# TensorSpeech/TensorFlowASR

Measured on AMD Instinct MI355X. Metric: audio-hours/sec (train step) Conformer-M RNN-T, higher is better.
Workload: dtype bf16; 1 GPU; Conformer-M transducer full train step (fwd+RNN-T loss+bwd+Adam), LibriSpeech-shaped 16 kHz utterances, 32/GPU, padding=batch, SpecAugment on, dropout 0.1; global_batch=32, parallelism=dp1, params=32461288

## Files before the change

include/tfasr_hip.h:

```cpp
#ifndef TFASR_HIP_H_
#define TFASR_HIP_H_

#include <stddef.h>
#include <stdint.h>

#ifdef __cplusplus
extern "C" {
#endif

#define TFASR_ABI_VERSION 44

typedef enum {
  TFASR_STATUS_SUCCESS = 0,
  TFASR_STATUS_INVALID_VALUE = 1,
  TFASR_STATUS_EXECUTION_FAILED = 2,
  TFASR_STATUS_UNSUPPORTED = 3
} tfasr_status_t;

typedef enum { TFASR_F32 = 0, TFASR_BF16 = 1 } tfasr_dtype_t;

const char* tfasr_status_string(int status);
int tfasr_abi_version(void);
size_t tfasr_launch_count(void);

// ... 8 lines not shown
int tfasr_rnnt_row_labels(const int32_t* labels, const int32_t* label_len, const int32_t* logit_len, const long* cell_off,
                          long total_cells, int B, int T, int U1, int V, int32_t* row_label, void* stream);
int tfasr_rnnt_loss_packed_stats(const void* logits, void* grads, const int32_t* labels, const int32_t* label_len,
                                 const int32_t* logit_len, const float* grad_scale, const long* cell_off, long total_cells,
                                 const float* lse_part, int lse_parts, const float* pick, int B, int T, int U1, int V, int blank,
                                 int dtype, float* costs, void* workspace, size_t workspace_bytes, void* stream);
int tfasr_rnnt_loss_packed(const void* logits, void* grads, const int32_t* labels, const int32_t* label_len,
                           const int32_t* logit_len, const float* grad_scale, const long* cell_off, long total_cells, int B,
                           int T, int U1, int V, int blank, int dtype, float* costs, void* workspace,
                           size_t workspace_bytes, void* stream);

int tfasr_ctc_loss_workspace_size(int B, int T, int U, int V, size_t* bytes);
int tfasr_ctc_loss(const void* logits, void* grads, const int32_t* labels, const int32_t* label_len,
                   const int32_t* logit_len, const float* grad_scale, int B, int T, int U, int V, int blank, int dtype,
                   float* costs, void* workspace, size_t workspace_bytes, void* stream);
int tfasr_ctc_greedy_decode(const void* logits, const int32_t* logit_len, int32_t* workspace_argmax, int32_t* tokens,
                            int32_t* tokens_len, int B, int T, int V, int blank, int dtype, void* stream);
int tfasr_ctc_greedy_decode_detail(const void* logits, const int32_t* logit_len, int32_t* workspace, int32_t* tokens, int32_t* tokens_len,
                                   int32_t* starts, int32_t* ends, float* tok_logp, float* tok_entropy, float* score, int B, int T, int V,
                                   int blank, int dtype, void* stream);

typedef enum { TFASR_ACT_NONE = 0, TFASR_ACT_SWISH = 1, TFASR_ACT_TANH = 2, TFASR_ACT_SIGMOID = 3, TFASR_ACT_TANH_OUT = 4,
               TFASR_ACT_FACTOR = 5  } tfasr_act_t;

typedef struct {
  const void* A; const void* B; void* D;
  const float* bias;
  const void* res;
  const void* dact_z;
  void* prez;
  int M, N, K;
  int lda, ldb, ldd;
  int trans_a, trans_b;
  int nb1, nb2;
  long sA1, sA2, sB1, sB2, sD1, sD2;
  float alpha, beta;
  int act;
  int dact;
  int dtype;
  int out_f32;
  int accumulate;
  int split_k;
  float drop_p;
  long drop_seed;
  float* ws;
  long ws_elems;
  float* colsum;
  float* lse_part; int lse_parts; const int32_t* row_label; float* pick;
  const long* seg_a_off; const long* seg_b_off; int seg_k;
  const float* rgrad_coef;
  const void* bns_x; const float* bns_fin; float* bns_out; int bns_copies;
  int bns_c;
  const int32_t* row_tiles; int n_row_tiles;
} tfasr_gemm_args;

int tfasr_gemm(const tfasr_gemm_args* args, void* stream);
int tfasr_gemm_group(const tfasr_gemm_args* args, int n, void* stream);

int tfasr_layernorm_fwd(const void* x, const float* gamma, const float* beta, void* y, float* mean, float* rstd,
                        long rows, int C, float eps, int dtype, void* stream);
int tfasr_ffn_fused_fwd(const void* x, const float* gamma, const float* beta, const void* W1, const float* b1, const void* W2,
                        const float* b2, void* y, void* ln, float* mean, float* rstd, void* z, void* h, long rows, int d, int F,
                        float ln_eps, float res_factor, float drop_p, long drop_seed1, long drop_seed2, int dtype, void* stream);
int tfasr_ffn_fused_fwd2(const void* x, const float* gamma, const float* beta, const void* W1, const float* b1, const void* W2,
                         const float* b2, void* y, void* ln, float* mean, float* rstd, void* z, int z_factor, void* h, long rows, int d, int F,
                         float ln_eps, float res_factor, float drop_p, long drop_seed1, long drop_seed2, int dtype, void* stream);
int tfasr_ln_dense_fwd(const void* x, const float* gamma, const float* beta, const void* W, const float* b, void* out, void* ln, float* mean,
                       float* rstd, long rows, int d, int N, float ln_eps, int dtype, void* stream);
int tfasr_layernorm_bwd(const void* dy, const void* x, const float* gamma, const float* mean, const float* rstd,
                        const void* add, void* dx, float* dgamma, float* dbeta, long rows, int C, int dtype,
                        void* stream);
int tfasr_layernorm_bwd_drop(const void* dy, const void* x, const float* gamma, const float* mean, const float* rstd,
                             const void* add, void* dx, float* dgamma, float* dbeta, void* dx_dropped, float drop_p,
                             long drop_seed, long rows, int C, int dtype, void* stream);
int tfasr_layernorm_bwd_part_blocks(long rows, int C, int dtype);
int tfasr_layernorm_bwd_part(const void* dy, const void* x, const float* gamma, const float* mean, const float* rstd, const void* add,
                             void* dx, float* part, void* dx_dropped, float drop_p, long drop_seed, long rows, int C, int dtype,
                             void* stream);
int tfasr_layernorm_bwd_part_n(const void* dy, const void* x, const float* gamma, const float* mean, const float* rstd, const void* add,
                               void* dx, float* part, int nblk, void* dx_dropped, float drop_p, long drop_seed, long rows, int C, int dtype,
                               void* stream);
int tfasr_dense_ln_bwd(const void* dy, const void* W, int K, const void* x, const float* gamma, const float* mean, const float* rstd,
                       const void* add, void* dx, float* part, int nblk, void* dx_dropped, float drop_p, long drop_seed, long rows,
                       int d, float alpha, int dtype, void* stream);
int tfasr_layernorm_bwd_fold(const float* part, int nsets, int nblk, int C, float* const* dgamma, float* const* dbeta, void* stream);
int tfasr_layernorm_bwd_fold_sets(const float* const* part, int nsets, int nblk, int C, float* const* dgamma, float* const* dbeta,
                                  void* stream);
int tfasr_bn_stats(const void* x, float* stats, long rows, int C, int dtype, void* stream);
int tfasr_bn_finalize(const float* stats, float count, const float* gamma, const float* beta, float* fin,
                      float* moving_mean, float* moving_var, float momentum, float eps, int C, int training,
                      void* stream);
int tfasr_bn_finalize_apply_fwd(const void* x, const float* stats, float count, const float* gamma, const float* beta, float* fin,
                                float* moving_mean, float* moving_var, float momentum, float eps, void* y, long rows, int C, int act,
                                int training, int dtype, void* stream);
int tfasr_bn_finalize_apply_fwd_copies(const void* x, const float* stats, int copies, float count, const float* gamma, const float* beta, float* fin,
                                       float* moving_mean, float* moving_var, float momentum, float eps, void* y, long rows, int C, int act,
                                       int training, int dtype, void* stream);
int tfasr_bn_apply_fwd(const void* x, const float* fin, void* y, long rows, int C, int act, int dtype, void* stream);
int tfasr_bn_bwd_stats(const void* x, const void* dy, const float* fin, float* bstats, long rows, int C, int act,
                       int dtype, void* stream);
int tfasr_bn_apply_bwd_grads(const void* x, const void* dy, const float* fin, const float* bstats, float count, void* dx, long rows,
                            int C, int act, float* dgamma, float* dbeta, float grad_scale, int dtype, void* stream);
int tfasr_bn_apply_bwd_grads_copies(const void* x, const void* dy, const float* fin, const float* bstats, int copies, float count, void* dx,
                                    long rows, int C, int act, float* dgamma, float* dbeta, float grad_scale, int dtype, void* stream);
int tfasr_bn_apply_bwd(const void* x, const void* dy, const float* fin, const float* bstats, float count, void* dx,
                       long rows, int C, int act, int dtype, void* stream);
// ... 111 lines not shown
                         void* stream);
int tfasr_decode_step(const float* emb, const float* lstm_k, const float* lstm_rk, const float* lstm_b, const float* ln_g,
                      const float* ln_b, const float* joint_pred_w, const float* joint_pred_b, const float* vocab_w,
                      const float* vocab_b, const float* packed, const float* encj, const int32_t* nframes, const int32_t* frame_idx,
                      const int32_t* tok_idx, const int32_t* prev_tok, const float* h, const float* c, int32_t* active,
                      float* h_new, float* c_new, float* z, float* logits, int B, int T, int E, int P, int J, int V,
                      int max_tokens, int mode, float ln_eps, void* stream);
int tfasr_decode_steps(const float* emb, const float* lstm_k, const float* lstm_rk, const float* lstm_b, const float* ln_g,
                       const float* ln_b, const float* joint_pred_w, const float* joint_pred_b, const float* vocab_w,
                       const float* vocab_b, const float* packed, const float* encj, const int32_t* nframes, int32_t* frame_idx,
                       int32_t* tok_idx, int32_t* prev_tok, float* h, float* c, int32_t* active, float* h_new, float* c_new, float* z,
                       float* logits, int32_t* tokens, int32_t* per_frame, int B, int T, int E, int P, int J, int V, int max_tokens,
                       int blank, int mode, int max_tokens_per_frame, float ln_eps, int iters, void* stream);
size_t tfasr_decode_pack_floats(int E, int P, int J, int V);
int tfasr_decode_pack(const float* emb, const float* lstm_k, const float* lstm_rk, const float* joint_pred_w, const float* vocab_w,
                      float* packed, int E, int P, int J, int V, void* stream);
int tfasr_decode_update(const void* logits, const int32_t* active, const int32_t* nframes, int32_t* frame_idx,
                        int32_t* prev_tok, int32_t* tok_idx, int32_t* tokens, int32_t* per_frame, const void* h_new,
                        const float* c_new, void* h, float* c, int B, int V, int P, int max_tokens, int blank, int mode,
                        int max_tokens_per_frame, int dtype, void* stream);
int tfasr_decode_update_detail(const void* logits, const int32_t* active, const int32_t* nframes, int32_t* frame_idx,
                               int32_t* prev_tok, int32_t* tok_idx, int32_t* tokens, int32_t* per_frame, const void* h_new,
                               const float* c_new, void* h, float* c, int32_t* tok_frames, float* tok_logp, float* tok_entropy, int B,
                               int V, int P, int max_tokens, int blank, int mode, int max_tokens_per_frame, int dtype, void* stream);
int tfasr_decode_steps_detail(const float* emb, const float* lstm_k, const float* lstm_rk, const float* lstm_b, const float* ln_g,
                              const float* ln_b, const float* joint_pred_w, const float* joint_pred_b, const float* vocab_w,
                              const float* vocab_b, const float* packed, const float* encj, const int32_t* nframes, int32_t* frame_idx,
                              int32_t* tok_idx, int32_t* prev_tok, float* h, float* c, int32_t* active, float* h_new, float* c_new,
                              float* z, float* logits, int32_t* tokens, int32_t* per_frame, int32_t* tok_frames, float* tok_logp,
                              float* tok_entropy, int B, int T, int E, int P, int J, int V, int max_tokens, int blank, int mode,
                              int max_tokens_per_frame, float ln_eps, int iters, void* stream);

int tfasr_conv1_fwd(const void* x, const float* w, const float* bias, void* y, int B, int T0, int F0, int C, int dtype,
                    void* stream);
int tfasr_conv1_bwd_weight(const void* x, const void* dy, float* dw, float* db, int B, int T0, int F0, int C,
                           int dtype, void* stream);
int tfasr_conv1_fwd_s2d(const void* x, const float* w, const float* bias, void* y, int B, int T0, int F0, int C, int dtype,
                        void* stream);
int tfasr_conv1_bwd_weight_s2d(const void* x, const void* dy, float* dw, float* db, int B, int T0, int F0, int C, int dtype,
                               void* stream);
int tfasr_conv1_stats(const void* x, const float* w, const float* bias, float* stats, int B, int T0, int F0, int C, int dtype,
                      void* stream);
int tfasr_conv1_bn_apply_s2d(const void* x, const float* w, const float* bias, const float* fin, void* y, int B, int T0, int F0, int C,
                             int dtype, void* stream);
int tfasr_conv1_bn_bwd_stats_s2d(const void* x, const float* w, const float* bias, const float* fin, const void* dy, float* bstats, int B,
                                 int T0, int F0, int C, int dtype, void* stream);
int tfasr_conv1_bn_bwd_apply_s2d(const void* x, const float* w, const float* bias, const float* fin, const float* bstats, float count,
                                 const void* dy, float* dw, float* db, int B, int T0, int F0, int C, int dtype, void* stream);
#define TFASR_CONV1_GRAM_DOUBLES 768
int tfasr_conv1_gram(const void* x, double* gram, int B, int T0, int F0, int dtype, void* stream);
int tfasr_conv1_stats_from_gram(const double* gram, const float* w, const float* bias, float* stats, int C, void* stream);
int tfasr_conv1_bn_bwd_onepass_s2d(const void* x, const float* w, const float* bias, const float* fin, const void* dy, float* bstats,
                                   float* pbuf, int B, int T0, int F0, int C, int dtype, void* stream);
int tfasr_conv1_bn_bwd_finalize(const double* gram, const float* w, const float* bias, const float* fin, const float* bstats, float count,
                                const float* pbuf, float* dw, float* db, int C, void* stream);
int tfasr_halo_zero(void* x, int B, int T2, int F2, int W, int dtype, void* stream);
int tfasr_s2d_edge_zero(void* x, int B, int T1, int F1, int C, int dtype, void* stream);
int tfasr_s2d_tail_fill(void* x, const int32_t* tiles, int n_tiles, const int32_t* rep_tt, int B, int T2, int F2, int C, int dtype,
                        void* stream);
int tfasr_im2col_3x3s2(const void* x, void* col, int B, int T1, int F1, int C, int dtype, void* stream);
int tfasr_col2im_3x3s2(const void* dcol, void* dx, int B, int T1, int F1, int C, int dtype, void* stream);

int tfasr_logmel(const float* signal, int B, int N, float preemph, const float* window, int frame_len, int frame_step,
                 int nfft, const float* melw, const int32_t* band, int F, float eps, void* out, int T0, int dtype,
                 void* stream);

int tfasr_rows_subsample_fwd(const void* x, void* y, int B, int T, int C, int stride, int dtype, void* stream);
int tfasr_rows_subsample_bwd(const void* dy, void* dx, int B, int T, int C, int stride, int dtype, void* stream);
int tfasr_se_pool(const void* x, const int32_t* lengths, float* pool, int B, int T, int C, int dtype, void* stream);
int tfasr_se_scale_fwd(const void* x, const float* scale, void* y, int B, int T, int C, int dtype, void* stream);
int tfasr_se_scale_bwd_reduce(const void* x, const void* dy, float* dscale, int B, int T, int C, int dtype, void* stream);
int tfasr_se_bwd_apply(const void* dy, const float* scale, const float* dpool, const int32_t* lengths, void* dx, int B, int T,
                       int C, int dtype, void* stream);
int tfasr_add_act_fwd(const void* a, const void* b, void* y, long n, int act, int dtype, void* stream);
int tfasr_add_act_bwd(const void* a, const void* b, const void* dy, void* d, long n, int act, int dtype, void* stream);

int tfasr_ctc_beam_search_host(const float* logits, const int32_t* logit_len, int B, int T, int V, int beam_width,
                               int blank_index, int32_t* tokens, int32_t* tokens_len, float* log_prob);

int tfasr_ctc_beam_search_workspace_size(int B, int T, int V, int beam_width, size_t* bytes);
int tfasr_ctc_beam_search(const void* logits, const int32_t* logit_len, int B, int T, int V, int beam_width, int top_paths,
                          int blank_index, int dtype, int32_t* tokens, int32_t* tokens_len, float* log_prob, void* workspace,
                          size_t workspace_bytes, void* stream);

int tfasr_rnnt_beam_workspace_size(int B, int T, int U, int J, int V, int beam_width, size_t* bytes);
int tfasr_rnnt_beam_search(const float* emb, const float* lstm_k, const float* lstm_rk, const float* lstm_b, const float* ln_g,
                           const float* ln_b, const float* joint_pred_w, const float* joint_pred_b, const float* vocab_w,
                           const float* vocab_b, const float* packed, const float* encj, const int32_t* nframes,
                           const int32_t* init_tok, const float* init_h, const float* init_c, int B, int T, int E, int U, int J,
                           int V, int beam_width, int top_paths, int blank, float ln_eps, int32_t* tokens, int32_t* tokens_len,
                           float* score, int32_t* next_tok, float* next_h, float* next_c, void* workspace, size_t workspace_bytes,
                           void* stream);
int tfasr_rnnt_beam_begin(const int32_t* init_tok, int B, int T, int U, int J, int V, int beam_width, int blank, void* workspace,
                          size_t workspace_bytes, void* stream);
int tfasr_rnnt_beam_select(const float* logits, const int32_t* nframes, int t, int B, int T, int U, int J, int V, int beam_width,
                           int blank, void* workspace, size_t workspace_bytes, void* stream);
int tfasr_rnnt_beam_nbest(int B, int T, int U, int J, int V, int beam_width, int top_paths, int blank, int32_t* tokens,
                          int32_t* tokens_len, float* score, void* workspace, size_t workspace_bytes, void* stream);

int tfasr_rnnt_beam_reset(const int32_t* mask, int B, int Tcap, int U, int J, int V, int beam_width, int blank, void* workspace,
                          size_t workspace_bytes, void* stream);
int tfasr_rnnt_beam_advance(const float* emb, const float* lstm_k, const float* lstm_rk, const float* lstm_b, const float* ln_g,
                            const float* ln_b, const float* joint_pred_w, const float* joint_pred_b, const float* vocab_w,
                            const float* vocab_b, const float* packed, const float* encj, const int32_t* nvalid, int B, int C,
                            int Tcap, int E, int U, int J, int V, int beam_width, int blank, float ln_eps, int frames_max_after,
                            void* workspace, size_t workspace_bytes, void* stream);
int tfasr_rnnt_beam_commit(const int32_t* final_mask, int32_t* committed, int32_t* tokens, int32_t* ntokens, int B, int Tcap, int U,
                           int J, int V, int beam_width, int width, int blank, void* workspace, size_t workspace_bytes, void* stream);
int tfasr_rnnt_beam_nbest_states(int B, int Tcap, int U, int J, int V, int beam_width, int top_paths, int blank, int width,
                                 int32_t* tokens, int32_t* tokens_len, float* score, int32_t* next_tok, float* next_h, float* next_c,
                                 void* workspace, size_t workspace_bytes, void* stream);
int tfasr_ctc_beam_stream_workspace_size(int B, int C, int Tcap, int V, int beam_width, size_t* bytes);
// ... 186 lines not shown
```

tensorflowasr_amd/_lib.py:

```python
import ctypes
import os
from ctypes import POINTER, Structure, c_char_p, c_float, c_int, c_int32, c_long, c_size_t, c_void_p

HERE = os.path.dirname(os.path.abspath(__file__))
LIB_PATH = os.environ.get("TFASR_LIB") or os.path.join(HERE, "lib", "libtfasr_hip.so")

TFASR_F32, TFASR_BF16 = 0, 1
ACT_NONE, ACT_SWISH, ACT_TANH, ACT_SIGMOID, ACT_TANH_OUT, ACT_FACTOR = 0, 1, 2, 3, 4, 5


class TfasrError(RuntimeError):
    pass


class GemmArgs(Structure):
    _fields_ = [
        ("A", c_void_p), ("B", c_void_p), ("D", c_void_p),
        ("bias", c_void_p), ("res", c_void_p), ("dact_z", c_void_p), ("prez", c_void_p),
        ("M", c_int), ("N", c_int), ("K", c_int),
        ("lda", c_int), ("ldb", c_int), ("ldd", c_int),
        ("trans_a", c_int), ("trans_b", c_int),
        ("nb1", c_int), ("nb2", c_int),
        ("sA1", c_long), ("sA2", c_long), ("sB1", c_long), ("sB2", c_long), ("sD1", c_long), ("sD2", c_long),
        ("alpha", c_float), ("beta", c_float),
        ("act", c_int), ("dact", c_int), ("dtype", c_int), ("out_f32", c_int), ("accumulate", c_int), ("split_k", c_int),
        ("drop_p", c_float), ("drop_seed", c_long),
        ("ws", c_void_p), ("ws_elems", c_long), ("colsum", c_void_p),
        ("lse_part", c_void_p), ("lse_parts", c_int), ("row_label", c_void_p), ("pick", c_void_p),
        ("seg_a_off", c_void_p), ("seg_b_off", c_void_p), ("seg_k", c_int),
        ("rgrad_coef", c_void_p),
        ("bns_x", c_void_p), ("bns_fin", c_void_p), ("bns_out", c_void_p), ("bns_copies", c_int), ("bns_c", c_int),
        ("row_tiles", c_void_p), ("n_row_tiles", c_int),
    ]


BLOCK_PARAM_NAMES = [
    "ff1/ln/g", "ff1/ln/b", "ff1/d1/w", "ff1/d1/b", "ff1/d2/w", "ff1/d2/b",
    "ff2/ln/g", "ff2/ln/b", "ff2/d1/w", "ff2/d1/b", "ff2/d2/w", "ff2/d2/b",
    "mhsa/ln/g", "mhsa/ln/b", "mhsa/qkv/w", "mhsa/qkv/b", "mhsa/pos/w", "mhsa/pos/b", "mhsa/o/w", "mhsa/o/b", "/enc/u", "/enc/v",
    "conv/ln/g", "conv/ln/b", "conv/pw1/w", "conv/pw1/b", "conv/dw/w", "conv/dw/b", "conv/bn/g", "conv/bn/b", "conv/pw2/w", "conv/pw2/b",
    "ln/g", "ln/b",
]
PHASE_A, PHASE_B = 1, 2


class BlockCfg(Structure):
    _fields_ = [
        ("B", c_int), ("T", c_int), ("d", c_int), ("H", c_int), ("dh", c_int), ("dff", c_int), ("ksize", c_int),
        ("dtype", c_int), ("training", c_int), ("save", c_int), ("use_mask", c_int), ("force_unfused", c_int), ("world", c_int),
        ("site0", c_int), ("drop_epoch", c_long),
        ("drop_p", c_float), ("ffm_res", c_float), ("mhsa_res", c_float), ("conv_res", c_float), ("ln_eps", c_float), ("bn_eps", c_float),
        ("bn_momentum", c_float),
        ("chunk_size", c_int), ("history_size", c_int), ("dw_norm_layer", c_int), ("dh_logical", c_int),
    ]


class BlockParams(Structure):
    _fields_ = [
        ("flat", c_void_p), ("shadow", c_void_p), ("grad", c_void_p), ("bn_mm", c_void_p), ("bn_mv", c_void_p), ("pe", c_void_p),
        ("off", c_long * len(BLOCK_PARAM_NAMES)),
    ]


class BlockIO(Structure):
    _fields_ = [
        ("x_in", c_void_p), ("x_out", c_void_p), ("dy", c_void_p), ("dx", c_void_p), ("lengths", c_void_p),
        ("bn_stats", c_void_p), ("bn_bstats", c_void_p),
        ("stash", c_void_p), ("stash_bytes", c_size_t), ("scratch", c_void_p), ("scratch_bytes", c_size_t),
        ("prezeroed", c_int), ("dpext_zero", c_void_p), ("wgrad_slot", c_int),
        ("pext_pre", c_void_p), ("defer_pos_grad", c_int), ("ln_part_ext", c_void_p), ("ln_part_ext_floats", c_size_t),
        ("dcv_keep", c_void_p), ("ds_keep", c_void_p), ("qv_keep", c_void_p), ("bn_stats_copies", c_int),
    ]


def _parse_header():
    import re

    hdr = os.path.join(HERE, "..", "include", "tfasr_hip.h")
    if not os.path.exists(hdr):
        hdr = os.path.join(HERE, "tfasr_hip.h")
    src = open(hdr).read()
    src = re.sub(r"/\*.*?\*/", "", src, flags=re.S)
    src = re.sub(r"typedef\s+struct\s*\{.*?\}\s*\w+\s*;", "", src, flags=re.S)
    sigs = {}
    for m in re.finditer(r"(const\s+char\s*\*|int|size_t)\s+(tfasr_[a-z0-9_]+)\s*\(([^)]*)\)\s*;", src):
# ... 75 lines not shown
```

tensorflowasr_amd/conformer.py:

```python
import math
import os

import numpy as np
import torch

from . import kernels as K
from .base_model import BaseModel
from .kernels import ACT_NONE, ACT_SWISH, ACT_TANH_OUT
from .params import ParamStore
from .schemas import AlignOutput, PredictInput, PredictOutput, RecognizeOutput, TrainData, TrainInput, TrainOutput


class SingleProcess:

    world = 1
    rank = 0

    def allreduce_stats_(self, t):
        return t

    def set_reduce(self, on):
        pass

    def grads_ready(self, lo, hi):
        pass

    def finish_grads(self):
        pass


def _split_k(M, N, Kd):
    tiles = -(-M // 128) * -(-N // 128)
    if tiles >= 512 or Kd <= 2048:
        return 1
    v = int(max(1, min(-(-1024 // tiles), Kd // 1024, 64)))
    return (v + 4) // 8 * 8 if v >= 12 else v


class ConformerTransducer(BaseModel):
    def __init__(self, cfg, device=None, dtype=torch.bfloat16, seed=0, dp=None):
        if not torch.cuda.is_available():
            raise K._lib.TfasrError("ConformerTransducer needs an MI355X (HIP) device; there is no CPU fallback")
        self.cfg = cfg
        self.device = torch.device("cuda", torch.cuda.current_device()) if device is None else torch.device(device)
        self.dtype = dtype
        pad = (dtype == torch.bfloat16 and cfg.head_size < 64 and getattr(cfg, "encoder", "conformer") == "conformer"
               and os.environ.get("TFASR_HEAD_PAD", "1") != "0")
        cpad = (dtype == torch.bfloat16 and cfg.filters % 64 != 0 and getattr(cfg, "encoder", "conformer") == "conformer"
                and getattr(cfg, "sub_norm", "batch") == "batch" and os.environ.get("TFASR_FILTER_PAD", "1") != "0")
        self.ps = ParamStore(cfg, self.device, dtype, seed, head_phys=64 if pad else None, filt_phys=-(-cfg.filters // 64) * 64 if cpad else None)
        self.dp = dp or SingleProcess()
        self.blank = cfg.blank
        self.time_reduction_factor = cfg.time_reduction_factor
        self.step = 0
        self._consts = {}
        self._bn1_sums_in_gemm = True
        self._bn_stats_copies = 8
        self._conv1_gram = True
        self._sub_tail_once = os.environ.get("TFASR_SUB_TAIL", "1") != "0"
        self._front_tail = None
        self._rng = np.random.default_rng([seed + 1000, int(self.dp.rank)])
        prio = -1
        self.pred_stream = torch.cuda.Stream(device=self.device, priority=prio)
        self.use_pred_stream = os.environ.get("TFASR_NO_PRED_STREAM", "0") != "1"
        self._dp_force_split = os.environ.get("TFASR_DP_FORCE_SPLIT", "0") == "1" and not isinstance(self.dp, SingleProcess)
        self._lstm_persist_auto = os.environ.get("TFASR_LSTM_PERSIST") is None
        self.optimizer = dict(beta1=0.9, beta2=0.98, eps=1e-9, weight_decay=1e-6, schedule=dict(
            dmodel=cfg.dmodel, warmup_steps=10000, scale=2.0, max_lr=0.05 / math.sqrt(cfg.dmodel)))
        self.ga_steps = 1
        self.prefetched_inputs = False
        self._ga_count = 0
        self._drop_epoch = 0
        self.native_blocks = os.environ.get("TFASR_NATIVE_BLOCK", "1") != "0"
        self.wgrad_stream = {"0": False, "1": True}.get(os.environ.get("TFASR_WGRAD_STREAM"), None)
        self._wgrad_keep = []
        self._blk_params, self._blk_sizes = {}, {}
        self._zero_pool = {}
        self.block_hoist = {"0": False, "1": True}.get(os.environ.get("TFASR_BLOCK_HOIST"), None)
        self.dpext_aux = True
        self.joint_wgrad_aux = False
        self._aux_pending = False
        if self.device.type != "cuda":
            self.aux_stream = None
        else:
            with torch.cuda.device(self.device):
                self.aux_stream = torch.cuda.ExternalStream(K.block_side_stream(), device=self.device)
        self._hoisted = {}
        self.fuse_joint_stats = True
        self.joint_recompute = os.environ.get("TFASR_JOINT_RECOMPUTE", "0") == "1"
        self._after_encoder = "pred/emb" if cfg.head == "transducer" else "dec/logits/w"
        self.timers = None
        self.timer_work = {}
        self.time_sections = False
        self.decode_precision = os.environ.get("TFASR_DECODE_PRECISION", "f32")
        self.decode_fused = True
        self._twin = None

    def _frontend_consts(self):
        if "fe" not in self._consts:
            c = self.cfg
            n = c.frame_length
            window = (0.5 - 0.5 * np.cos(2.0 * np.pi * np.arange(n) / n)).astype(np.float32)
            melw = _mel_weight_matrix(c.num_feature_bins, c.nfft // 2 + 1, c.sample_rate, c.lower_edge_hertz, c.upper_edge_hertz)
            band = np.zeros((melw.shape[1], 2), np.int32)
            for m in range(melw.shape[1]):
                nz = np.nonzero(melw[:, m])[0]
                band[m] = (nz[0], nz[-1]) if len(nz) else (0, -1)
            dev = self.device
            self._consts["fe"] = (torch.from_numpy(window).to(dev), torch.from_numpy(melw).to(dev), torch.from_numpy(band).to(dev))
        return self._consts["fe"]

    def _pe_ext(self, T):
# ... 28 lines not shown
        K.gemm(x, dy, ps.g2d(wname), din, dout, rows, x.stride(0), dy.stride(0), dout, trans_a=True, accumulate=True,
               split_k=_split_k(din, dout, rows), alpha=alpha, colsum=ps.g(bname) if bname is not None else None)
        if not need_dx:
            return None
        return K.matmul(dy, W, trans_b=True, alpha=alpha, dact_z=dact_z, dact=dact, drop_p=drop[0], drop_seed=drop[1])

    def _h2d(self, x, dtype=torch.int32):
        t = x if isinstance(x, torch.Tensor) else torch.as_tensor(np.asarray(x))
        t = t.to(dtype)
        if t.device.type == "cpu":
            if self.device.type == "cuda":
                t = t.pin_memory()
            t = t.to(self.device, non_blocking=True)
        return t

    def frontend(self, signals, signals_length, training=False, masks=None):
        c = self.cfg
        window, melw, band = self._frontend_consts()
        feats = K.logmel(signals, window, melw, band, c.frame_step, c.nfft, c.preemphasis, c.epsilon, self.dtype)
        flen = [-(-int(n) // c.frame_step) for n in signals_length]
        if training:
            if masks is None:
                masks = self.draw_specaugment(flen)
            fm, tm = masks
            if fm is not None or tm is not None:
                K.specaugment(feats, None if fm is None else self._h2d(fm), None if tm is None else self._h2d(tm), 0.0)
        self._front_tail = (feats, self._feature_tail(signals_length, masks[1] if training else None))
        return feats, flen

    def _feature_tail(self, signals_length, tm):
        step = self.cfg.frame_step
        tf = -(-(np.asarray([int(n) for n in signals_length], dtype=np.int64) + 1) // step)
        if tm is not None:
            if not isinstance(tm, torch.Tensor) or tm.device.type != "cpu":
                return None
            m = tm.numpy().astype(np.int64)
            if m.shape[1] > 0:
                tf = np.maximum(tf, (m[:, :, 0] + m[:, :, 1]).max(axis=1))
        return tuple(int(v) for v in tf)

    @staticmethod
    def _tail_rows(tf, T0):
        tf = np.asarray(tf, dtype=np.int64)
        t1c = (tf + 1) // 2 + 1
        a1 = (t1c + 1) // 2 + 1
        return dict(feats=tf, a1=a1, o=a1 + 1, a2=a1 + 1)

    @classmethod
    def _tail_blocks(cls, tf, B, T0, T2, F2):
        rep = cls._tail_rows(tf, T0)["o"]
        has = rep + 1 <= T2
        rep = np.where(has, rep, 1)
        end = np.where(has, rep + 1, T2 + 1)
        nblk = -(-(B * (T2 + 1) * (F2 + 1)) // 256)
        base = np.arange(B, dtype=np.int64) * (T2 + 1)
        lo = (base + 1) * (F2 + 1) // 256
        hi = ((base + end) * (F2 + 1) - 1) // 256
        mark = np.zeros(nblk + 1, np.int64)
        np.add.at(mark, lo, 1)
        np.add.at(mark, hi + 1, -1)
        real = np.cumsum(mark[:nblk]) > 0
        return np.flatnonzero(real), np.flatnonzero(~real), rep

    def _tail_tables(self, tf, B, T0, T2, F2):
        key = ("tail", tf, T0, F2)
        hit = self._consts.get(key, 0)
        if hit != 0:
            return hit
        comp, skip, rep = self._tail_blocks(tf, B, T0, T2, F2)
        out = None
        if skip.size * 16 >= comp.size + skip.size:
            dev = self._h2d(np.concatenate([comp, skip, rep]).astype(np.int32))
            out = (dev[:comp.size], dev[comp.size:comp.size + skip.size], dev[comp.size + skip.size:])
        old = [k for k in self._consts if isinstance(k, tuple) and k[:1] == ("tail",)]
        for k in old[:max(0, len(old) - 7)]:
            del self._consts[k]
        self._consts[key] = out
        return out

    def draw_specaugment(self, flen):
        c = self.cfg
        fcfg, tcfg = c.freq_masking, c.time_masking
        B = len(flen)
        rng = self._rng
        nf = fcfg.get("num_masks", 0) if fcfg else 0
        nt = tcfg.get("num_masks", 0) if tcfg else 0
        fm = np.zeros((B, nf, 2), np.int32) if nf > 0 else None
        tm = np.zeros((B, nt, 2), np.int32) if nt > 0 else None
        nb = c.num_feature_bins
        rnd, rint = rng.random, rng.integers
        fprob = fcfg.get("prob", 1.0) if fcfg else 1.0
        fmax = max(1, int(fcfg["mask_factor"])) if nf > 0 else 1
        tprob = tcfg.get("prob", 1.0) if tcfg else 1.0
        tup = np.float32(tcfg.get("p_upperbound", 1.0)) if tcfg else np.float32(1.0)
        for b in range(B):
            ln = int(flen[b])
            for k in range(nf):
                do = 1 if rnd() <= fprob else 0
                f = do * min(int(rint(0, fmax)), nb)
                fm[b, k] = (do * int(rint(0, max(1, nb - f))), f)
            if nt > 0:
                Tb = max(1, int(math.floor(np.float32(ln) * tup)))
            for k in range(nt):
                do = 1 if rnd() <= tprob else 0
                t = do * min(int(rint(0, Tb)), ln)
                tm[b, k] = (do * int(rint(0, max(1, ln - t))), t)
        return (None if fm is None else torch.from_numpy(fm)), (None if tm is None else torch.from_numpy(tm))

    def _zeros_f32(self, n):
        n = (n + 63) // 64 * 64
        size = max(1 << 18, n)
        arena, cur = self._consts.get("zero_arena", (None, 0))
        if arena is None or cur + n > arena.numel():
            arena, cur = torch.zeros(size, dtype=torch.float32, device=self.device), 0
        self._consts["zero_arena"] = (arena, cur + n)
        return arena[cur:cur + n]

    def _bn_fwd(self, x2d, name, training, act, rows=None, y=None):
        ps = self.ps
        C = x2d.shape[1]
        fin = torch.empty(4 * C, dtype=torch.float32, device=self.device)
        if training:
            stats = self._zeros_f32(2 * C + 1)[:2 * C + 1]
            K.bn_stats(x2d, stats)
            count = (x2d.shape[0] if rows is None else rows) * self.dp.world
            self.dp.allreduce_stats_(stats[:2 * C])
# ... 23 lines not shown
            return False
        return self.dtype == torch.float32 or self.ps.filt_phys % 64 == 0

    def _salloc(self, rows, width, slack, tag=None):
        key = ("salloc", tag, rows, width, slack)
        if tag is not None and slack > 0 and key in self._consts:
            full = self._consts[key]
        else:
            full = torch.empty((rows + 2 * slack) * width, dtype=self.dtype, device=self.device)
            if slack > 0:
                full[:slack * width].zero_()
                full[(slack + rows) * width:].zero_()
                if tag is not None:
                    old = [k for k in self._consts if isinstance(k, tuple) and k[:2] == ("salloc", tag)]
                    for k in old[:max(0, len(old) - 3)]:
                        del self._consts[k]
                    self._consts[key] = full
        return full, full[slack * width:(slack + rows) * width].view(rows, width)

    def _seg_tables(self, F2, C):
        key = ("seg", F2, C)
        if key not in self._consts:
            shift, blk = [], []
            for kh, kw in self._SEG:
                dt, pt = (-1, kh) if kh < 2 else (0, 0)
                df, pf = (-1, kw) if kw < 2 else (0, 0)
                shift.append(dt * (F2 + 1) + df)
                blk.append(pt * 2 + pf)
            dev = self.device
            nck = C // 64 if C % 64 == 0 else 1
            ck = C // nck
            order = sorted(range(9), key=lambda i: (blk[i], i))
            fwd_a = torch.tensor([shift[i] * 4 * C + blk[i] * C + cc * ck for cc in range(nck) for i in order], dtype=torch.int64, device=dev)
            fwd_b = torch.tensor([(i * C + cc * ck) * C for cc in range(nck) for i in order], dtype=torch.int64, device=dev)
            dgrad = {}
            for b in range(4):
                segs = [i for i in range(9) if blk[i] == b]
                dgrad[b] = (segs, torch.tensor([-shift[i] * C + cc * ck for cc in range(nck) for i in segs], dtype=torch.int64, device=dev),
                            torch.tensor([i * C * C + cc * ck for cc in range(nck) for i in segs], dtype=torch.int64, device=dev))
            self._consts[key] = (shift, blk, (fwd_a, fwd_b, ck), dgrad)
        return self._consts[key]

    def _subsampling_fwd_s2d(self, feats, flen, training, ctx):
        ps, c = self.ps, self.cfg
        B, T0, F0 = feats.shape
        C = ps.filt_phys
        T1, F1 = (T0 + 1) // 2, (F0 + 1) // 2
        T2, F2 = (T1 + 1) // 2, (F1 + 1) // 2
        rows, slack = B * (T2 + 1) * (F2 + 1), F2 + 2
        shift, blk, fwd_a, _ = self._seg_tables(F2, C)
        w0, b0 = ps.p("enc/sub/conv0/w"), ps.p("enc/sub/conv0/b")
        fin0 = torch.empty(4 * C, dtype=torch.float32, device=self.device)
        nm = "enc/sub/bn0"
        gram = None
        if training:
            stats = self._zeros_f32(2 * C + 1)[:2 * C + 1]
            if self._conv1_gram:
                gram = K.conv1_gram(feats, torch.empty(K.CONV1_GRAM_DOUBLES, dtype=torch.float64, device=self.device))
                K.conv1_stats_from_gram(gram, w0, b0, stats)
            else:
                K.conv1_stats(feats, w0, b0, stats)
            count0 = B * T1 * F1 * self.dp.world
            self.dp.allreduce_stats_(stats[:2 * C])
            K.bn_finalize(stats, count0, ps.p(nm + "/g"), ps.p(nm + "/b"), fin0, ps.state[nm + "/mm"], ps.state[nm + "/mv"], 0.99, 1e-3, True)
        else:
            count0 = B * T1 * F1
            K.bn_finalize(None, 1, ps.p(nm + "/g"), ps.p(nm + "/b"), fin0, ps.state[nm + "/mm"], ps.state[nm + "/mv"], 0.99, 1e-3, False)
        a1_full, a1 = self._salloc(rows, 4 * C, slack, tag="a1")
        K.conv1_bn_apply_s2d(feats, w0, b0, fin0, a1)
        K.halo_zero(a1, B, T2, F2, 4 * C)
        K.s2d_edge_zero(a1, B, T1, F1, C)
        bn0 = (fin0, count0, gram)
        W = ps.w2d("enc/sub/conv1/w")
        _, o = self._salloc(rows, C, slack, tag="o")
        if self.dtype == torch.float32:
            flat, base = a1_full, slack * 4 * C
            for i in range(9):
                K.gemm(flat[base + shift[i] * 4 * C + blk[i] * C:], W[i * C:(i + 1) * C], o, rows, C, C, 4 * C, C, C,
                       bias=ps.p("enc/sub/conv1/b") if i == 0 else None, accumulate=i > 0)
        else:
            tail, ft, self._front_tail = None, self._front_tail, None
            if self._sub_tail_once and ft is not None and ft[0] is feats and ft[1] is not None and len(ft[1]) == B:
                tail = self._tail_tables(ft[1], B, T0, T2, F2)
            if tail is not None:
                try:
                    K.gemm(a1, W, o, rows, C, 9 * C, 4 * C, C, C, bias=ps.p("enc/sub/conv1/b"), seg=fwd_a, row_tiles=tail[0])
                    K.s2d_tail_fill(o, tail[1], tail[2], B, T2, F2, C)
                except K._lib.TfasrUnsupported:
                    tail = None
            if tail is None:
                K.gemm(a1, W, o, rows, C, 9 * C, 4 * C, C, C, bias=ps.p("enc/sub/conv1/b"), seg=fwd_a)
        K.halo_zero(o, B, T2, F2, C)
        _, a2 = self._salloc(rows, C, 0)
        _, bn1 = self._bn_fwd(o, "enc/sub/bn1", training, ACT_SWISH, rows=B * T2 * F2, y=a2)
        K.halo_zero(a2, B, T2, F2, C)
        drop = self._drop(0, training)
        d = c.dmodel
        x0 = torch.empty(B * T2, d, dtype=self.dtype, device=self.device)
        a2flat = a2.view(-1)
        K.gemm(a2flat[((F2 + 1) + 1) * C:], ps.w2d("enc/linear/w"), x0, T2, d, F2 * C, (F2 + 1) * C, d, d, bias=ps.p("enc/linear/b"),
               nb1=B, sA=((T2 + 1) * (F2 + 1) * C, 0), sD=(T2 * d, 0), drop_p=drop[0], drop_seed=drop[1])
        elen = [-(-(-(-n // 2)) // 2) for n in flen]
        if ctx is not None:
            ctx["sub"] = dict(s2d=True, feats=feats, bn0=bn0, a1=a1, a1_full=a1_full, o=o, bn1=bn1, a2=a2,
                              dims=(B, T0, F0, T1, F1, T2, F2), drop=drop)
        return x0, T2, elen

    def _subsampling_bwd_s2d(self, dx0, ctx):
        ps, c = self.ps, self.cfg
        s = ctx["sub"]
        B, T0, F0, T1, F1, T2, F2 = s["dims"]
        C, d = ps.filt_phys, c.dmodel
        rows, slack = B * (T2 + 1) * (F2 + 1), F2 + 2
        shift, blk, _, dgrad = self._seg_tables(F2, C)
        dx0m = self._mask_grad(dx0, s["drop"])
        dx0h = torch.zeros(B, T2 + 1, d, dtype=self.dtype, device=self.device)
        dx0h[:, 1:].copy_(dx0m.view(B, T2, d))
        dx0h = dx0h.view(B * (T2 + 1), d)
        a2flat = s["a2"].view(-1)
        K.gemm(a2flat[C:], dx0h, ps.g2d("enc/linear/w"), F2 * C, d, B * (T2 + 1), (F2 + 1) * C, d, d, trans_a=True, accumulate=True,
               split_k=_split_k(F2 * C, d, B * (T2 + 1)), colsum=ps.g("enc/linear/b"))
        _, da2 = self._salloc(rows, C, 0)
        bst, ncp = None, 8
        if self._bn1_sums_in_gemm and self.dtype == torch.bfloat16 and C % 8 == 0 and 256 % (C // 8) == 0 and 64 <= C <= 2048:
            bst = self._zeros_f32(ncp * 2 * C)[:ncp * 2 * C].view(ncp, 2 * C)
            try:
                K.gemm(dx0h, ps.w2d("enc/linear/w"), da2.view(-1)[C:], B * (T2 + 1), F2 * C, d, d, d, (F2 + 1) * C, trans_b=True,
                       bns=(s["o"].view(-1)[C:], s["bn1"][0], bst, C))
            except K._lib.TfasrUnsupported:
                bst = None
        if bst is None:
            K.gemm(dx0h, ps.w2d("enc/linear/w"), da2.view(-1)[C:], B * (T2 + 1), F2 * C, d, d, d, (F2 + 1) * C, trans_b=True)
        K.halo_zero(da2, B, T2, F2, C)
        do_full, do = self._salloc(rows, C, slack, tag="do")
        if bst is None:
            self._bn_bwd(s["o"], da2, "enc/sub/bn1", s["bn1"], ACT_SWISH, dx=do)
        else:
            fin1, count1 = s["bn1"]
            self.dp.allreduce_stats_(bst.view(-1))
            K.bn_apply_bwd(s["o"], da2, fin1, bst, count1, ACT_SWISH, dx=do, dgamma=ps.g("enc/sub/bn1/g"), dbeta=ps.g("enc/sub/bn1/b"),
                           grad_scale=1.0 / self.dp.world, copies=ncp)
        K.halo_zero(do, B, T2, F2, C)
        a1_full, base = s["a1_full"], slack * 4 * C
        gW = ps.g2d("enc/sub/conv1/w")
        calls = []
        for i in range(9):
            calls.append(dict(A=a1_full[base + shift[i] * 4 * C + blk[i] * C:], B=do, out=gW[i * C:(i + 1) * C], M=C, N=C, K=rows, lda=4 * C, ldb=C,
                              ldd=C, trans_a=True, accumulate=True, split_k=_split_k(C, C, rows), colsum=ps.g("enc/sub/conv1/b") if i == 0 else None))
        K.gemm_group(calls)
        W = ps.w2d("enc/sub/conv1/w")
        _, da1 = self._salloc(rows, 4 * C, 0)
        dobase = slack * C
        for b4 in range(4):
            segs, a_off, b_off = dgrad[b4]
            out = da1.view(-1)[b4 * C:]
            if self.dtype == torch.float32:
                for j, i in enumerate(segs):
                    K.gemm(do_full[dobase - shift[i] * C:], W[i * C:(i + 1) * C], out, rows, C, C, C, C, 4 * C, trans_b=True, accumulate=j > 0)
            else:
                K.gemm(do, W, out, rows, C, len(segs) * C, C, C, 4 * C, trans_b=True, seg=(a_off, b_off, C // (a_off.numel() // len(segs))))
        fin0, count0, gram = s["bn0"]
        w0, b0 = ps.p("enc/sub/conv0/w"), ps.p("enc/sub/conv0/b")
        if gram is not None:
            zz = self._zeros_f32(12 * C)
            bstats, pbuf = zz[:2 * C], zz[2 * C:12 * C]
            K.conv1_bn_bwd_onepass_s2d(s["feats"], w0, b0, fin0, da1, bstats, pbuf)
            self.dp.allreduce_stats_(bstats)
            K.conv1_bn_bwd_finalize(gram, w0, b0, fin0, bstats, count0, pbuf, ps.g("enc/sub/conv0/w"), ps.g("enc/sub/conv0/b"))
        else:
            bstats = torch.zeros(2 * C, dtype=torch.float32, device=self.device)
            K.conv1_bn_bwd_stats_s2d(s["feats"], w0, b0, fin0, da1, bstats)
            self.dp.allreduce_stats_(bstats)
            K.conv1_bn_bwd_apply_s2d(s["feats"], w0, b0, fin0, bstats, count0, da1, ps.g("enc/sub/conv0/w"), ps.g("enc/sub/conv0/b"))
        inv = 1.0 / self.dp.world
        K.axpy(ps.g("enc/sub/bn0/b"), bstats[:C].contiguous(), inv)
        K.axpy(ps.g("enc/sub/bn0/g"), bstats[C:].contiguous(), inv)

    def _sub_norm_fwd(self, x2d, name, training):
        if self.cfg.sub_norm == "layer":
            yn, mean, rstd = K.layernorm_fwd(x2d, self.ps.p(name + "/g"), self.ps.p(name + "/b"))
            return K.add_act_fwd(yn, None, ACT_SWISH), (yn, mean, rstd)
        return self._bn_fwd(x2d, name, training, ACT_SWISH)

    def _sub_norm_bwd(self, x2d, dy2d, name, saved):
        if self.cfg.sub_norm == "layer":
            yn, mean, rstd = saved
            dyn = K.add_act_bwd(yn, None, dy2d, ACT_SWISH)
            return K.layernorm_bwd(dyn, x2d, self.ps.p(name + "/g"), mean, rstd, self.ps.g(name + "/g"), self.ps.g(name + "/b"))
        return self._bn_bwd(x2d, dy2d, name, saved, ACT_SWISH)

    def _subsampling_fwd(self, feats, flen, training, ctx):
        if self._s2d_enabled():
            return self._subsampling_fwd_s2d(feats, flen, training, ctx)
        ps, c = self.ps, self.cfg
        B, T0, F0 = feats.shape
        C = ps.filt_phys
        c1 = K.conv1_fwd(feats, ps.p("enc/sub/conv0/w"), ps.p("enc/sub/conv0/b"))
        T1, F1 = c1.shape[1], c1.shape[2]
        a1, bn0 = self._sub_norm_fwd(c1.view(-1, C), "enc/sub/bn0", training)
        a1 = a1.view(B, T1, F1, C)
        col = K.im2col_3x3s2(a1)
        T2, F2 = (T1 + 1) // 2, (F1 + 1) // 2
        c2 = K.matmul(col, ps.w2d("enc/sub/conv1/w"), bias=ps.p("enc/sub/conv1/b"))
        a2, bn1 = self._sub_norm_fwd(c2, "enc/sub/bn1", training)
        merged = a2.view(B * T2, F2 * C)
        drop = self._drop(0, training)
        x0 = K.matmul(merged, ps.w2d("enc/linear/w"), bias=ps.p("enc/linear/b"), drop_p=drop[0], drop_seed=drop[1])
        elen = [-(-(-(-n // 2)) // 2) for n in flen]
        if ctx is not None:
            ctx["sub"] = dict(feats=feats, c1=c1, bn0=bn0, col=col, c2=c2, bn1=bn1, merged=merged, dims=(B, T0, F0, T1, F1, T2, F2), drop=drop)
        return x0, T2, elen

    def _subsampling_bwd(self, dx0, ctx):
        if ctx["sub"].get("s2d"):
            return self._subsampling_bwd_s2d(dx0, ctx)
        ps, c = self.ps, self.cfg
        s = ctx["sub"]
        B, T0, F0, T1, F1, T2, F2 = s["dims"]
        C = ps.filt_phys
# ... 1172 lines not shown
```

tensorflowasr_amd/csrc/conv2d.hip:

```cpp
#include "common.h"
#include <type_traits>
#include <algorithm>

namespace {

inline int flat_grid(long n) { return (int)std::max<long>(1, std::min<long>((n + 255) / 256, 256L * 32)); }

__device__ __forceinline__ long s2d_off(int b, int t, int f, int T2, int F2, int C) {
  return ((((long)b * (T2 + 1) + (t >> 1) + 1) * (F2 + 1) + (f >> 1) + 1) * 4 + ((t & 1) * 2 + (f & 1))) * C;
}

template <typename T>
__global__ __launch_bounds__(256) void conv1_fwd_kernel(const T* __restrict__ x, const float* __restrict__ w,
                                                        const float* __restrict__ bias, T* __restrict__ y, int B, int T0,
                                                        int F0, int T1, int F1, int C, int s2d) {
  const int c8n = C / 8;
  const long n8 = (long)B * T1 * F1 * c8n;
  const long i0 = (long)blockIdx.x * blockDim.x + threadIdx.x;
  const long stride = (long)gridDim.x * blockDim.x;
  const int c = (int)(i0 % c8n) * 8;
  float wr[9][8], br[8];
#pragma unroll
  for (int k = 0; k < 8; ++k) br[k] = bias ? bias[c + k] : 0.f;
#pragma unroll
// ... 197 lines not shown
}

template <typename T>
__global__ __launch_bounds__(256) void col2im_kernel(const T* __restrict__ dcol, T* __restrict__ dx, int B, int T1,
                                                     int F1, int T2, int F2, int C) {
  const int c8n = C / 8;
  const long n8 = (long)B * T1 * F1 * c8n;
  for (long i = (long)blockIdx.x * blockDim.x + threadIdx.x; i < n8; i += (long)gridDim.x * blockDim.x) {
    const int c = (int)(i % c8n) * 8;
    long r = i / c8n;
    const int f1 = (int)(r % F1); r /= F1;
    const int t1 = (int)(r % T1);
    const int b = (int)(r / T1);
    float acc[8] = {0, 0, 0, 0, 0, 0, 0, 0};
#pragma unroll
    for (int kh = 0; kh < 3; ++kh) {
      const int tt = t1 + 2 - kh;
      if (tt < 0 || (tt & 1)) continue;
      const int t2 = tt >> 1;
      if (t2 >= T2) continue;
#pragma unroll
      for (int kw = 0; kw < 3; ++kw) {
        const int ff = f1 + 2 - kw;
        if (ff < 0 || (ff & 1)) continue;
        const int f2 = ff >> 1;
        if (f2 >= F2) continue;
        float v[8];
        ld8(dcol + ((((long)b * T2 + t2) * F2 + f2) * 9 + kh * 3 + kw) * C + c, v);
#pragma unroll
        for (int k = 0; k < 8; ++k) acc[k] += v[k];
      }
    }
    st8(dx + i * 8, acc);
  }
}

template <int N> __device__ __forceinline__ void ldn(const float* p, float (&v)[N]) {
#pragma unroll
  for (int k = 0; k < N; k += 4) { const float4 a = *reinterpret_cast<const float4*>(p + k); v[k] = a.x; v[k + 1] = a.y; v[k + 2] = a.z; v[k + 3] = a.w; }
}
template <int N> __device__ __forceinline__ void ldn(const bf16_t* p, float (&v)[N]) {
#pragma unroll
  for (int k = 0; k < N; k += 4) {
    const uint2 a = *reinterpret_cast<const uint2*>(p + k);
    v[k] = __uint_as_float(a.x << 16); v[k + 1] = __uint_as_float(a.x & 0xffff0000u); v[k + 2] = __uint_as_float(a.y << 16); v[k + 3] = __uint_as_float(a.y & 0xffff0000u);
  }
}
typedef __attribute__((ext_vector_type(2))) float c1f2_t;
__device__ __forceinline__ c1f2_t c1fma(c1f2_t a, c1f2_t b, c1f2_t c) { return __builtin_elementwise_fma(a, b, c); }
template <typename T, int MODE, int CPT>
__global__ __launch_bounds__(256) void conv1_bn_kernel(const T* __restrict__ x, const float* __restrict__ w, const float* __restrict__ bias,
                                                       const float* __restrict__ fin, const float* __restrict__ bstats, float inv_count,
                                                       T* __restrict__ y, const T* __restrict__ dy, float* __restrict__ out0,
                                                       float* __restrict__ out1, int B, int T0, int F0, int T1, int F1, int C) {
  extern __shared__ float sm[];
  float* xs = sm;
  float* red = sm + 3 * (F0 + 2);
  constexpr int NQ = MODE == 3 ? 10 : (MODE == 4 ? 11 : 2);
  constexpr int CP2 = CPT / 2;
  static_assert(CPT % 2 == 0, "channel pairs");
  const int cgn = C / CPT, FS = 256 / cgn;
  const int cg = threadIdx.x % cgn, fs = threadIdx.x / cgn;
  const bool on = fs < FS;
  const int c = cg * CPT;
  const int T2 = (T1 + 1) / 2, F2 = (F1 + 1) / 2;
  c1f2_t wr[9][CP2], br[CP2];
#pragma unroll
  for (int k = 0; k < CP2; ++k) br[k] = bias ? c1f2_t{bias[c + 2 * k], bias[c + 2 * k + 1]} : c1f2_t{0.f, 0.f};
#pragma unroll
  for (int tap = 0; tap < 9; ++tap)
#pragma unroll
    for (int k = 0; k < CP2; ++k) wr[tap][k] = c1f2_t{w[tap * C + c + 2 * k], w[tap * C + c + 2 * k + 1]};
  c1f2_t mean[CP2], rstd[CP2], sc[CP2], sh[CP2], s0[CP2], s1[CP2];
  if (MODE >= 1) {
#pragma unroll
    for (int k = 0; k < CP2; ++k) {
      mean[k] = c1f2_t{fin[c + 2 * k], fin[c + 2 * k + 1]}; rstd[k] = c1f2_t{fin[C + c + 2 * k], fin[C + c + 2 * k + 1]};
      sc[k] = c1f2_t{fin[2 * C + c + 2 * k], fin[2 * C + c + 2 * k + 1]}; sh[k] = c1f2_t{fin[3 * C + c + 2 * k], fin[3 * C + c + 2 * k + 1]};
    }
  }
  if (MODE == 3) {
#pragma unroll
    for (int k = 0; k < CP2; ++k) {
      s0[k] = c1f2_t{bstats[c + 2 * k] * inv_count, bstats[c + 2 * k + 1] * inv_count};
      s1[k] = c1f2_t{bstats[C + c + 2 * k] * inv_count, bstats[C + c + 2 * k + 1] * inv_count};
    }
  }
  c1f2_t acc2[NQ][CP2];
#pragma unroll
  for (int q = 0; q < NQ; ++q)
#pragma unroll
    for (int k = 0; k < CP2; ++k) acc2[q][k] = c1f2_t{0.f, 0.f};
  const int nrows = B * T1;
  for (int row = blockIdx.x; row < nrows; row += gridDim.x) {
    const int b = row / T1, t = row - b * T1;
    __syncthreads();
    for (int i = threadIdx.x; i < 3 * (F0 + 2); i += 256) {
      const int kh = i / (F0 + 2), fi = i - kh * (F0 + 2) - 2, ti = 2 * t + kh - 2;
      xs[i] = (ti >= 0 && ti < T0 && fi >= 0 && fi < F0) ? Num<T>::ld(x + ((long)b * T0 + ti) * F0 + fi) : 0.f;
    }
    __syncthreads();
    if (!on) continue;
    auto body = [&](int f, const float (&dr)[CPT]) {
      c1f2_t a[CP2];
      float xv[9];
#pragma unroll
      for (int kh = 0; kh < 3; ++kh)
#pragma unroll
        for (int kw = 0; kw < 3; ++kw) xv[kh * 3 + kw] = xs[kh * (F0 + 2) + 2 * f + kw];
#pragma unroll
      for (int k = 0; k < CP2; ++k) a[k] = br[k];
#pragma unroll
      for (int tap = 0; tap < 9; ++tap) {
        const c1f2_t x2 = c1f2_t{xv[tap], xv[tap]};
#pragma unroll
        for (int k = 0; k < CP2; ++k) a[k] = c1fma(wr[tap][k], x2, a[k]);
      }
      if (MODE == 0) {
#pragma unroll
        for (int k = 0; k < CP2; ++k) { acc2[0][k] += a[k]; acc2[1][k] = c1fma(a[k], a[k], acc2[1][k]); }
      } else if (MODE == 1) {
        float o[CPT];
#pragma unroll
        for (int k = 0; k < CP2; ++k) {
          const c1f2_t z = c1fma(a[k], sc[k], sh[k]);
          o[2 * k] = swishf_(z[0]); o[2 * k + 1] = swishf_(z[1]);
        }
        static_assert(MODE != 1 || CPT == 8, "apply pass: 8 channels per thread");
        if constexpr (CPT == 8) st8(y + s2d_off(b, t, f, T2, F2, C) + c, o);
      } else {
        c1f2_t d[CP2];
#pragma unroll
        for (int k = 0; k < CP2; ++k) {
          const c1f2_t z = c1fma(a[k], sc[k], sh[k]);
          const c1f2_t dz = c1f2_t{dr[2 * k] * dswishf_(z[0]), dr[2 * k + 1] * dswishf_(z[1])};
          const c1f2_t xh = (a[k] - mean[k]) * rstd[k];
          if (MODE == 2 || MODE == 4) { acc2[0][k] += dz; acc2[1][k] = c1fma(dz, xh, acc2[1][k]); }
          d[k] = (MODE == 3) ? sc[k] * (dz - s0[k] - xh * s1[k]) : dz;
        }
        if (MODE == 4) {
#pragma unroll
          for (int tap = 0; tap < 9; ++tap) {
            const c1f2_t x2 = c1f2_t{xv[tap], xv[tap]};
#pragma unroll
            for (int k = 0; k < CP2; ++k) acc2[2 + tap][k] = c1fma(d[k], x2, acc2[2 + tap][k]);
          }
        }
// ... 162 lines not shown
    dw[k * C + c] += (float)(sc * ((double)pbuf[k * C + c] - s0 * sk - s1 * X));
  }
  if (db) db[c] += (float)(sc * ((double)pbuf[9 * C + c] - s0 * N - s1 * rstd * (ws + N * (b - mean))));
}

template <typename T>
__global__ __launch_bounds__(256) void halo_zero_kernel(T* __restrict__ x, int B, int T2, int F2, int W) {
  const int w8 = W / 8, per_b = (F2 + 1) + T2;
  const long n = (long)B * per_b * w8;
  const float z[8] = {0, 0, 0, 0, 0, 0, 0, 0};
  for (long i = (long)blockIdx.x * blockDim.x + threadIdx.x; i < n; i += (long)gridDim.x * blockDim.x) {
    const int c8 = (int)(i % w8);
    long r = i / w8;
    const int k = (int)(r % per_b), b = (int)(r / per_b);
    const int tt = k <= F2 ? 0 : k - F2, ff = k <= F2 ? k : 0;
    st8(x + (((long)b * (T2 + 1) + tt) * (F2 + 1) + ff) * W + (long)c8 * 8, z);
  }
}
template <typename T>
__global__ __launch_bounds__(256) void s2d_edge_zero_kernel(T* __restrict__ x, int B, int T1, int F1, int T2, int F2, int C) {
  const int c8n = C / 8;
  const int nt = (T1 & 1) ? F2 * 2 : 0;
  const int nf = (F1 & 1) ? T2 * 2 : 0;
  const long n = (long)B * (nt + nf) * c8n;
  const float z[8] = {0, 0, 0, 0, 0, 0, 0, 0};
  for (long i = (long)blockIdx.x * blockDim.x + threadIdx.x; i < n; i += (long)gridDim.x * blockDim.x) {
    const int c8 = (int)(i % c8n);
    long r = i / c8n;
    const int k = (int)(r % (nt + nf)), b = (int)(r / (nt + nf));
    int tt, ff, blk;
    if (k < nt) { tt = T2; ff = 1 + (k >> 1); blk = 2 + (k & 1); }
    else { const int q = k - nt; tt = 1 + (q >> 1); ff = F2; blk = (q & 1) * 2 + 1; }
    st8(x + ((((long)b * (T2 + 1) + tt) * (F2 + 1) + ff) * 4 + blk) * C + (long)c8 * 8, z);
  }
}

__global__ __launch_bounds__(256) void s2d_tail_fill_kernel(uint4* __restrict__ x, const int32_t* __restrict__ tiles, const int32_t* __restrict__ rep_tt,
                                                            int T2, int F2, int c8n, long rows) {
  const long nblk = (rows + 255) / 256;
  const long tile = min(max((long)tiles[blockIdx.x >> 2], 0L), nblk - 1);
  const long r0 = tile * 256 + (blockIdx.x & 3) * 64;
  const int per_b = (T2 + 1) * (F2 + 1);
  for (int i = threadIdx.x; i < 64 * c8n; i += 256) {
    const long row = r0 + i / c8n;
    if (row >= rows) break;
    const int c8 = i % c8n;
    const int b = (int)(row / per_b), ff = (int)(row % (F2 + 1));
    const int rt = min(max(rep_tt[b], 1), T2);
    const long src = ((long)b * (T2 + 1) + rt) * (F2 + 1) + ff;
    if (src != row) x[row * c8n + c8] = x[src * c8n + c8];
  }
}

}

#define DISPATCH_T(dtype, CALL_F32, CALL_BF16) \
  do { if ((dtype) == TFASR_F32) { CALL_F32; } else if ((dtype) == TFASR_BF16) { CALL_BF16; } else return TFASR_STATUS_INVALID_VALUE; } while (0)

static int conv1_fwd_impl(const void* x, const float* w, const float* bias, void* y, int B, int T0, int F0, int C,
                          int dtype, void* stream_, int s2d) {
  if (!x || !w || !y || B <= 0 || T0 <= 0 || F0 <= 0 || C <= 0 || C % 8) return TFASR_STATUS_INVALID_VALUE;
  const int T1 = (T0 + 1) / 2, F1 = (F0 + 1) / 2;
  hipStream_t s = (hipStream_t)stream_;
  if (C == 256 && F0 + 2 <= 260) {
    const int g2 = std::min(B * T1, 8192);
    DISPATCH_T(dtype,
               TFASR_KLAUNCH(conv1_fwd_rows_kernel<float>, dim3(g2), dim3(256), 0, s, (const float*)x, w, bias, (float*)y, B, T0, F0, T1, F1, s2d),
               TFASR_KLAUNCH(conv1_fwd_rows_kernel<bf16_t>, dim3(g2), dim3(256), 0, s, (const bf16_t*)x, w, bias, (bf16_t*)y, B, T0, F0, T1, F1, s2d));
    TFASR_CHECK_LAUNCH();
    return TFASR_STATUS_SUCCESS;
  }
  int grid = flat_grid((long)B * T1 * F1 * C / 8);
  if ((256 % (C / 8)) != 0) {
    const int c8n = C / 8;
    grid = ((grid + c8n - 1) / c8n) * c8n;
  }
  DISPATCH_T(dtype,
             TFASR_KLAUNCH(conv1_fwd_kernel<float>, dim3(grid), dim3(256), 0, s, (const float*)x, w, bias, (float*)y, B, T0, F0, T1, F1, C, s2d),
             TFASR_KLAUNCH(conv1_fwd_kernel<bf16_t>, dim3(grid), dim3(256), 0, s, (const bf16_t*)x, w, bias, (bf16_t*)y, B, T0, F0, T1, F1, C, s2d));
  TFASR_CHECK_LAUNCH();
  return TFASR_STATUS_SUCCESS;
}

extern "C" int tfasr_conv1_fwd(const void* x, const float* w, const float* bias, void* y, int B, int T0, int F0, int C,
                               int dtype, void* stream_) {
  return conv1_fwd_impl(x, w, bias, y, B, T0, F0, C, dtype, stream_, 0);
}
extern "C" int tfasr_conv1_fwd_s2d(const void* x, const float* w, const float* bias, void* y, int B, int T0, int F0, int C,
                                   int dtype, void* stream_) {
  return conv1_fwd_impl(x, w, bias, y, B, T0, F0, C, dtype, stream_, 1);
}

static int conv1_bwd_weight_impl(const void* x, const void* dy, float* dw, float* db, int B, int T0, int F0, int C,
                                 int dtype, void* stream_, int s2d) {
  if (!x || !dy || !dw || B <= 0 || T0 <= 0 || F0 <= 0 || C <= 0 || C > 256 || (C % 8)) return TFASR_STATUS_INVALID_VALUE;
  const int T1 = (T0 + 1) / 2, F1 = (F0 + 1) / 2;
  hipStream_t s = (hipStream_t)stream_;
  if (C == 256 && F0 + 2 <= 260) {
    const int g2 = std::min(B * T1, 1024);
    DISPATCH_T(dtype,
               TFASR_KLAUNCH(conv1_bwd_weight_rows_kernel<float>, dim3(g2), dim3(256), 0, s, (const float*)x, (const float*)dy, dw, db, B, T0, F0, T1, F1, s2d),
               TFASR_KLAUNCH(conv1_bwd_weight_rows_kernel<bf16_t>, dim3(g2), dim3(256), 0, s, (const bf16_t*)x, (const bf16_t*)dy, dw, db, B, T0, F0, T1, F1, s2d));
    TFASR_CHECK_LAUNCH();
    return TFASR_STATUS_SUCCESS;
  }
  const long npos = (long)B * T1 * F1;
  const int grid = (int)std::max<long>(1, std::min<long>(npos / 64 + 1, 1024));
  DISPATCH_T(dtype,
             TFASR_KLAUNCH((conv1_bwd_weight_kernel<float, 32>), dim3(grid), dim3(256), 0, s, (const float*)x, (const float*)dy, dw, db, B, T0, F0, T1, F1, C, s2d),
             TFASR_KLAUNCH((conv1_bwd_weight_kernel<bf16_t, 32>), dim3(grid), dim3(256), 0, s, (const bf16_t*)x, (const bf16_t*)dy, dw, db, B, T0, F0, T1, F1, C, s2d));
  TFASR_CHECK_LAUNCH();
  return TFASR_STATUS_SUCCESS;
}

extern "C" int tfasr_conv1_bwd_weight(const void* x, const void* dy, float* dw, float* db, int B, int T0, int F0, int C,
                                      int dtype, void* stream_) {
  return conv1_bwd_weight_impl(x, dy, dw, db, B, T0, F0, C, dtype, stream_, 0);
}
extern "C" int tfasr_conv1_bwd_weight_s2d(const void* x, const void* dy, float* dw, float* db, int B, int T0, int F0, int C,
                                          int dtype, void* stream_) {
  return conv1_bwd_weight_impl(x, dy, dw, db, B, T0, F0, C, dtype, stream_, 1);
}

template <int MODE>
static int conv1_bn_launch(const void* x, const float* w, const float* bias, const float* fin, const float* bstats, float count, void* y,
                           const void* dy, float* out0, float* out1, int B, int T0, int F0, int C, int dtype, void* stream_) {
  if (!x || !w || B <= 0 || T0 <= 0 || F0 <= 0 || C <= 0 || C > 256 || (C % 8)) return TFASR_STATUS_INVALID_VALUE;
  constexpr int CPT = MODE >= 2 ? 4 : 8;
  constexpr int NQL = MODE == 3 ? 10 : (MODE == 4 ? 11 : 2);
  const int T1 = (T0 + 1) / 2, F1 = (F0 + 1) / 2;
  hipStream_t s = (hipStream_t)stream_;
  const size_t smem_q = (size_t)(3 * (F0 + 2) + NQL * C) * sizeof(float);
  static const int env_grid = 0;
  static int res_blocks[2] = {0, 0};
  static size_t res_smem[2] = {0, 0};
  const int di = dtype == TFASR_F32 ? 0 : 1;
  if (MODE != 1 && !env_grid && (res_blocks[di] == 0 || res_smem[di] != smem_q)) {
    int dev = 0, cus = 0, per = 0;
    hipError_t e = hipGetDevice(&dev);
    if (e == hipSuccess) e = hipDeviceGetAttribute(&cus, hipDeviceAttributeMultiprocessorCount, dev);
    if (e == hipSuccess)
      e = di == 0 ? hipOccupancyMaxActiveBlocksPerMultiprocessor(&per, conv1_bn_kernel<float, MODE, CPT>, 256, smem_q)
                  : hipOccupancyMaxActiveBlocksPerMultiprocessor(&per, conv1_bn_kernel<bf16_t, MODE, CPT>, 256, smem_q);
    res_blocks[di] = (e == hipSuccess && per > 0 && cus > 0) ? per * cus : 768;
    res_smem[di] = smem_q;
  }
  const int grid = std::min(B * T1, MODE == 1 ? 8192 : std::max(64, env_grid ? env_grid : res_blocks[di]));
  const size_t smem = (size_t)(3 * (F0 + 2) + NQL * C) * sizeof(float);
  const float inv = count > 0.f ? 1.f / count : 0.f;
  DISPATCH_T(dtype,
             TFASR_KLAUNCH((conv1_bn_kernel<float, MODE, CPT>), dim3(grid), dim3(256), smem, s, (const float*)x, w, bias, fin, bstats, inv, (float*)y,
                                (const float*)dy, out0, out1, B, T0, F0, T1, F1, C),
             TFASR_KLAUNCH((conv1_bn_kernel<bf16_t, MODE, CPT>), dim3(grid), dim3(256), smem, s, (const bf16_t*)x, w, bias, fin, bstats, inv, (bf16_t*)y,
                                (const bf16_t*)dy, out0, out1, B, T0, F0, T1, F1, C));
  TFASR_CHECK_LAUNCH();
  return TFASR_STATUS_SUCCESS;
}

extern "C" int tfasr_conv1_stats(const void* x, const float* w, const float* bias, float* stats, int B, int T0, int F0, int C, int dtype,
                                 void* stream_) {
  if (!stats) return TFASR_STATUS_INVALID_VALUE;
  return conv1_bn_launch<0>(x, w, bias, nullptr, nullptr, 0.f, nullptr, nullptr, stats, nullptr, B, T0, F0, C, dtype, stream_);
}
extern "C" int tfasr_conv1_bn_apply_s2d(const void* x, const float* w, const float* bias, const float* fin, void* y, int B, int T0, int F0,
                                        int C, int dtype, void* stream_) {
  if (!fin || !y) return TFASR_STATUS_INVALID_VALUE;
  return conv1_bn_launch<1>(x, w, bias, fin, nullptr, 0.f, y, nullptr, nullptr, nullptr, B, T0, F0, C, dtype, stream_);
}
extern "C" int tfasr_conv1_bn_bwd_stats_s2d(const void* x, const float* w, const float* bias, const float* fin, const void* dy, float* bstats,
                                            int B, int T0, int F0, int C, int dtype, void* stream_) {
  if (!fin || !dy || !bstats) return TFASR_STATUS_INVALID_VALUE;
  return conv1_bn_launch<2>(x, w, bias, fin, nullptr, 0.f, nullptr, dy, bstats, nullptr, B, T0, F0, C, dtype, stream_);
}
extern "C" int tfasr_conv1_bn_bwd_apply_s2d(const void* x, const float* w, const float* bias, const float* fin, const float* bstats,
                                            float count, const void* dy, float* dw, float* db, int B, int T0, int F0, int C, int dtype,
                                            void* stream_) {
  if (!fin || !bstats || !dy || !dw || count <= 0.f) return TFASR_STATUS_INVALID_VALUE;
  return conv1_bn_launch<3>(x, w, bias, fin, bstats, count, nullptr, dy, dw, db, B, T0, F0, C, dtype, stream_);
}

extern "C" int tfasr_conv1_gram(const void* x, double* gram, int B, int T0, int F0, int dtype, void* stream_) {
  if (!x || !gram || B <= 0 || T0 <= 0 || F0 <= 0) return TFASR_STATUS_INVALID_VALUE;
  const int T1 = (T0 + 1) / 2, F1 = (F0 + 1) / 2;
  hipStream_t s = (hipStream_t)stream_;
  if (hipMemsetAsync(gram, 0, GRAM_COPIES * GRAM_STRIDE * sizeof(double), s) != hipSuccess) return TFASR_STATUS_EXECUTION_FAILED;
  const int grid = std::max(1, std::min((B * T1 + 5) / 6, 1024));
  const size_t smem = (size_t)6 * 3 * (F0 + 2) * sizeof(float);
  DISPATCH_T(dtype, TFASR_KLAUNCH(conv1_gram_kernel<float>, dim3(grid), dim3(256), smem, s, (const float*)x, gram, B, T0, F0, T1, F1),
             TFASR_KLAUNCH(conv1_gram_kernel<bf16_t>, dim3(grid), dim3(256), smem, s, (const bf16_t*)x, gram, B, T0, F0, T1, F1));
  TFASR_CHECK_LAUNCH();
  return TFASR_STATUS_SUCCESS;
}
extern "C" int tfasr_conv1_stats_from_gram(const double* gram, const float* w, const float* bias, float* stats, int C, void* stream_) {
  if (!gram || !w || !stats || C <= 0) return TFASR_STATUS_INVALID_VALUE;
  TFASR_KLAUNCH(conv1_stats_from_gram_kernel, dim3((C + 255) / 256), dim3(256), 0, (hipStream_t)stream_, gram, w, bias, stats, C);
  TFASR_CHECK_LAUNCH();
  return TFASR_STATUS_SUCCESS;
}
extern "C" int tfasr_conv1_bn_bwd_onepass_s2d(const void* x, const float* w, const float* bias, const float* fin, const void* dy, float* bstats,
                                              float* pbuf, int B, int T0, int F0, int C, int dtype, void* stream_) {
  if (!fin || !dy || !bstats || !pbuf) return TFASR_STATUS_INVALID_VALUE;
  return conv1_bn_launch<4>(x, w, bias, fin, nullptr, 0.f, nullptr, dy, bstats, pbuf, B, T0, F0, C, dtype, stream_);
}
extern "C" int tfasr_conv1_bn_bwd_finalize(const double* gram, const float* w, const float* bias, const float* fin, const float* bstats,
                                           float count, const float* pbuf, float* dw, float* db, int C, void* stream_) {
  if (!gram || !w || !fin || !bstats || !pbuf || !dw || C <= 0 || count <= 0.f) return TFASR_STATUS_INVALID_VALUE;
  TFASR_KLAUNCH(conv1_bn_bwd_finalize_kernel, dim3((C + 255) / 256), dim3(256), 0, (hipStream_t)stream_, gram, w, bias, fin, bstats,
                     1.f / count, pbuf, dw, db, C);
  TFASR_CHECK_LAUNCH();
  return TFASR_STATUS_SUCCESS;
}

extern "C" int tfasr_halo_zero(void* x, int B, int T2, int F2, int W, int dtype, void* stream_) {
  if (!x || B <= 0 || T2 <= 0 || F2 <= 0 || W <= 0 || W % 8) return TFASR_STATUS_INVALID_VALUE;
  hipStream_t s = (hipStream_t)stream_;
  const int grid = flat_grid((long)B * ((F2 + 1) + T2) * (W / 8));
  DISPATCH_T(dtype, TFASR_KLAUNCH(halo_zero_kernel<float>, dim3(grid), dim3(256), 0, s, (float*)x, B, T2, F2, W),
             TFASR_KLAUNCH(halo_zero_kernel<bf16_t>, dim3(grid), dim3(256), 0, s, (bf16_t*)x, B, T2, F2, W));
  TFASR_CHECK_LAUNCH();
  return TFASR_STATUS_SUCCESS;
}

extern "C" int tfasr_s2d_edge_zero(void* x, int B, int T1, int F1, int C, int dtype, void* stream_) {
  if (!x || B <= 0 || T1 <= 0 || F1 <= 0 || C <= 0 || C % 8) return TFASR_STATUS_INVALID_VALUE;
  if (!(T1 & 1) && !(F1 & 1)) return TFASR_STATUS_SUCCESS;
  const int T2 = (T1 + 1) / 2, F2 = (F1 + 1) / 2;
  hipStream_t s = (hipStream_t)stream_;
  const int grid = flat_grid((long)B * (((T1 & 1) ? F2 * 2 : 0) + ((F1 & 1) ? T2 * 2 : 0)) * (C / 8));
  DISPATCH_T(dtype, TFASR_KLAUNCH(s2d_edge_zero_kernel<float>, dim3(grid), dim3(256), 0, s, (float*)x, B, T1, F1, T2, F2, C),
             TFASR_KLAUNCH(s2d_edge_zero_kernel<bf16_t>, dim3(grid), dim3(256), 0, s, (bf16_t*)x, B, T1, F1, T2, F2, C));
  TFASR_CHECK_LAUNCH();
  return TFASR_STATUS_SUCCESS;
}

extern "C" int tfasr_s2d_tail_fill(void* x, const int32_t* tiles, int n_tiles, const int32_t* rep_tt, int B, int T2, int F2, int C, int dtype,
                                   void* stream_) {
  if (!x || !tiles || !rep_tt || B <= 0 || T2 <= 0 || F2 <= 0 || C <= 0 || n_tiles < 0) return TFASR_STATUS_INVALID_VALUE;
  const long rows = (long)B * (T2 + 1) * (F2 + 1);
  if (n_tiles > (rows + 255) / 256) return TFASR_STATUS_INVALID_VALUE;
  if (dtype != TFASR_BF16 || C % 8 || (((uintptr_t)x) & 15)) return TFASR_STATUS_UNSUPPORTED;
  if (n_tiles == 0) return TFASR_STATUS_SUCCESS;
  TFASR_KLAUNCH(s2d_tail_fill_kernel, dim3(4 * n_tiles), dim3(256), 0, (hipStream_t)stream_, (uint4*)x, tiles, rep_tt, T2, F2, C / 8, rows);
  TFASR_CHECK_LAUNCH();
  return TFASR_STATUS_SUCCESS;
}

extern "C" int tfasr_im2col_3x3s2(const void* x, void* col, int B, int T1, int F1, int C, int dtype, void* stream_) {
  if (!x || !col || B <= 0 || T1 <= 0 || F1 <= 0 || C <= 0 || C % 8) return TFASR_STATUS_INVALID_VALUE;
  const int T2 = (T1 + 1) / 2, F2 = (F1 + 1) / 2;
  hipStream_t s = (hipStream_t)stream_;
  const int grid = flat_grid((long)B * T2 * F2 * 9 * C / 8);
  DISPATCH_T(dtype,
             TFASR_KLAUNCH(im2col_kernel<float>, dim3(grid), dim3(256), 0, s, (const float*)x, (float*)col, B, T1, F1, T2, F2, C),
             TFASR_KLAUNCH(im2col_kernel<bf16_t>, dim3(grid), dim3(256), 0, s, (const bf16_t*)x, (bf16_t*)col, B, T1, F1, T2, F2, C));
  TFASR_CHECK_LAUNCH();
  return TFASR_STATUS_SUCCESS;
}

extern "C" int tfasr_col2im_3x3s2(const void* dcol, void* dx, int B, int T1, int F1, int C, int dtype, void* stream_) {
  if (!dcol || !dx || B <= 0 || T1 <= 0 || F1 <= 0 || C <= 0 || C % 8) return TFASR_STATUS_INVALID_VALUE;
  const int T2 = (T1 + 1) / 2, F2 = (F1 + 1) / 2;
  hipStream_t s = (hipStream_t)stream_;
  const int grid = flat_grid((long)B * T1 * F1 * C / 8);
  DISPATCH_T(dtype,
             TFASR_KLAUNCH(col2im_kernel<float>, dim3(grid), dim3(256), 0, s, (const float*)dcol, (float*)dx, B, T1, F1, T2, F2, C),
             TFASR_KLAUNCH(col2im_kernel<bf16_t>, dim3(grid), dim3(256), 0, s, (const bf16_t*)dcol, (bf16_t*)dx, B, T1, F1, T2, F2, C));
  TFASR_CHECK_LAUNCH();
  return TFASR_STATUS_SUCCESS;
}
```

tensorflowasr_amd/csrc/gemm.hip:

```cpp
#include "common.h"
#include <stdlib.h>

namespace {

constexpr int BM = 128, BN = 128;

template <typename T> struct Cfg;
template <> struct Cfg<bf16_t> { static constexpr int BK = 64, LD = 72; };
template <> struct Cfg<float>  { static constexpr int BK = 16, LD = 17; };

__device__ __forceinline__ bool aligned16(const void* p) { return (((uintptr_t)p) & 15) == 0; }

__device__ __forceinline__ void load_direct(bf16_t* s, const bf16_t* g, long ld, int rows0, int nrows_total,
                                            int kt, int k_end) {
  constexpr int BK = Cfg<bf16_t>::BK, LD = Cfg<bf16_t>::LD;
  for (int c = threadIdx.x; c < BM * BK / 8; c += 256) {
    const int row = c / (BK / 8), kc = (c % (BK / 8)) * 8;
    const int gr = rows0 + row, gk = kt + kc;
    uint4 v = make_uint4(0, 0, 0, 0);
    if (gr < nrows_total) {
      const bf16_t* p = g + (long)gr * ld + gk;
      if (gk + 8 <= k_end && aligned16(p)) v = *reinterpret_cast<const uint4*>(p);
      else {
        uint32_t w[4] = {0, 0, 0, 0};
// ... 340 lines not shown
  return TFASR_STATUS_SUCCESS;
}

}

int tfasr_gemm_fast_try(const tfasr_gemm_args& a, hipStream_t stream);

static bool use_fast_path() {
  static int v = -1;
  if (v < 0) v = 1;
  return v == 1;
}

int tfasr_gemm_group_fast_try(const tfasr_gemm_args* a, int n, hipStream_t stream);

extern "C" int tfasr_gemm_group(const tfasr_gemm_args* args, int n, void* stream_) {
  if (!args || n <= 0) return TFASR_STATUS_INVALID_VALUE;
  static const bool off = false;
  int i = 0;
  while (i < n) {
    const int m = n - i < 10 ? n - i : 10;
    int st = TFASR_STATUS_UNSUPPORTED;
    if (!off && use_fast_path()) st = tfasr_gemm_group_fast_try(args + i, m, (hipStream_t)stream_);
    if (st == TFASR_STATUS_UNSUPPORTED) {
      for (int j = 0; j < m; ++j) {
        st = tfasr_gemm(args + i + j, stream_);
        if (st != TFASR_STATUS_SUCCESS) return st;
      }
    } else if (st != TFASR_STATUS_SUCCESS) {
      return st;
    }
    i += m;
  }
  return TFASR_STATUS_SUCCESS;
}

extern "C" int tfasr_gemm(const tfasr_gemm_args* args, void* stream_) {
  if (!args || !args->A || !args->B || (!args->D && !args->lse_part)) return TFASR_STATUS_INVALID_VALUE;
  tfasr_gemm_args a = *args;
  if (a.rgrad_coef && (!a.row_label || !a.D || a.lse_part)) return TFASR_STATUS_INVALID_VALUE;
  if (a.M <= 0 || a.N <= 0 || a.K <= 0) return TFASR_STATUS_INVALID_VALUE;
  if (a.nb1 < 1) a.nb1 = 1;
  if (a.nb2 < 1) a.nb2 = 1;
  if (a.split_k < 1) a.split_k = 1;
  if (a.accumulate && !a.out_f32) return TFASR_STATUS_INVALID_VALUE;
  if (a.split_k > 1 && !a.accumulate) return TFASR_STATUS_INVALID_VALUE;
  if (a.split_k > 1 && (a.res || a.dact_z || a.prez || a.act != TFASR_ACT_NONE || a.drop_p > 0.f)) return TFASR_STATUS_INVALID_VALUE;
  if (a.drop_p < 0.f || a.drop_p >= 1.f) return TFASR_STATUS_INVALID_VALUE;
  if (a.colsum && !(a.accumulate && a.trans_a && !a.trans_b && a.nb1 * a.nb2 == 1)) return TFASR_STATUS_INVALID_VALUE;
  if (a.row_tiles) {
    if (a.n_row_tiles <= 0 || a.n_row_tiles > (a.M + 255) / 256) return TFASR_STATUS_INVALID_VALUE;
    if (!a.seg_a_off || a.trans_a || a.accumulate || a.split_k > 1 || a.nb1 * a.nb2 != 1 || a.dtype != TFASR_BF16) return TFASR_STATUS_UNSUPPORTED;
  }
  hipStream_t stream = (hipStream_t)stream_;
  if (a.dtype == TFASR_BF16 && use_fast_path()) {
    const int st = tfasr_gemm_fast_try(a, stream);
    if (st != TFASR_STATUS_UNSUPPORTED) return st;
  }
  if (a.lse_part || a.rgrad_coef || a.bns_out) return TFASR_STATUS_UNSUPPORTED;
  if (a.seg_a_off) return TFASR_STATUS_UNSUPPORTED;
  if (a.colsum) {
    const int st = tfasr_colsum(a.B, a.ldb, a.colsum, a.K, a.N, a.alpha, a.dtype, stream_);
    if (st != TFASR_STATUS_SUCCESS) return st;
    a.colsum = nullptr;
  }
  if (a.dtype == TFASR_BF16) return launch<bf16_t>(a, stream);
  if (a.dtype == TFASR_F32) return launch<float>(a, stream);
  return TFASR_STATUS_INVALID_VALUE;
}
```

tensorflowasr_amd/csrc/gemm_fast.hip:

```cpp
#include "common.h"
#include <type_traits>
#include <string.h>
#include <stdlib.h>

typedef __attribute__((ext_vector_type(4))) short short4_t;

#ifdef TFASR_GEMM_TIMING
__device__ long long g_gemm_timing[16 * 32768];
#endif

namespace {

constexpr int BM = 128, BK = 64;
constexpr int A_BYTES = BM * BK * 2;

#define LDS_PTR(p) ((__attribute__((address_space(3))) void*)(p))
#define GLB_PTR(p) ((const __attribute__((address_space(1))) void*)(p))

__device__ __forceinline__ uint32_t lds_u32(const char* s) {
  return (uint32_t)__builtin_amdgcn_readfirstlane((int)(uint32_t)(uintptr_t)s);
}
__device__ __forceinline__ void glds16(const void* g, const char* lds_uniform) {
#ifdef TFASR_GLDS_BUILTIN
  __builtin_amdgcn_global_load_lds(GLB_PTR(g), LDS_PTR(lds_uniform), 16, 0, 0);
// ... 143 lines not shown
      else    b[kk][j] = frag_trans<BN_>(sB, wn * WN + j * 16, kk * 32 + g * 8, r);
    }
  }
  __builtin_amdgcn_sched_barrier(0);
  hook.reads_done();
#pragma unroll
  for (int kk = 0; kk < 2; ++kk)
#pragma unroll
    for (int i = 0; i < 4; ++i) {
#pragma unroll
      for (int j = 0; j < NJ; ++j) acc[i][j] = __builtin_amdgcn_mfma_f32_16x16x32_bf16(a[kk][i], b[kk][j], acc[i][j], 0, 0, 0);
      if constexpr (!std::is_same<Hook, NoHook>::value) {
        hook.between(kk * 4 + i);
        __builtin_amdgcn_sched_barrier(0);
      }
    }
  if constexpr (CS) {
    if (do_cs) {
      const short one = (short)0x3F80;
      const short8_t ones = {one, one, one, one, one, one, one, one};
#pragma unroll
      for (int kk = 0; kk < 2; ++kk)
#pragma unroll
        for (int j = 0; j < NJ; ++j) accb[j] = __builtin_amdgcn_mfma_f32_16x16x32_bf16(ones, b[kk][j], accb[j], 0, 0, 0);
    }
  }
}

__device__ __forceinline__ void unpack8(const uint4& a, float (&v)[8]) {
  v[0] = __uint_as_float(a.x << 16); v[1] = __uint_as_float(a.x & 0xffff0000u); v[2] = __uint_as_float(a.y << 16); v[3] = __uint_as_float(a.y & 0xffff0000u);
  v[4] = __uint_as_float(a.z << 16); v[5] = __uint_as_float(a.z & 0xffff0000u); v[6] = __uint_as_float(a.w << 16); v[7] = __uint_as_float(a.w & 0xffff0000u);
}
__device__ __forceinline__ float act_f(float v, int act) {
  switch (act) {
    case TFASR_ACT_SWISH: return swishf_(v);
    case TFASR_ACT_TANH: return tanhf(v);
    case TFASR_ACT_SIGMOID: return sigmoidf_(v);
    default: return v;
  }
}
__device__ __forceinline__ float dact_f(float z, int act) {
  switch (act) {
    case TFASR_ACT_SWISH: return dswishf_(z);
    case TFASR_ACT_TANH: { const float t = tanhf(z); return 1.f - t * t; }
    case TFASR_ACT_SIGMOID: { const float s = sigmoidf_(z); return s * (1.f - s); }
    case TFASR_ACT_TANH_OUT: return 1.f - z * z;
    case TFASR_ACT_FACTOR: return z;
    default: return 1.f;
  }
}

enum : int { E_ACT = 1 , E_DACT = 2 , E_DROP = 4, E_RES = 8, E_WS = 16 , E_CSUM = 32 , E_LSE = 64 , E_RGRAD = 128 , E_GEN = 256, E_BNS = 512 , E_MUL = 1024  };

template <bool TA, bool TB, int BN_, int EPI, int NST = 2, bool FIXED = false, bool SEG = false, bool ONE = false>
__device__ __forceinline__ void gemm_fast_body(const tfasr_gemm_args& p, const int gx, const int gy, const int gz, const int ntiles, const int bid, const int G) {
  constexpr bool GEN = (EPI & E_GEN) != 0;
  constexpr bool C_ACT = GEN || (EPI & E_ACT), C_DACT = GEN || (EPI & E_DACT), C_DROP = GEN || (EPI & E_DROP), C_RES = GEN || (EPI & E_RES);
  constexpr bool C_WS = (EPI & E_WS) != 0;
  constexpr bool C_CS = (EPI & E_CSUM) != 0;
  constexpr bool C_LSE = (EPI & E_LSE) != 0;
  constexpr bool C_BNS = (EPI & E_BNS) != 0;
  constexpr bool C_MUL = (EPI & E_MUL) != 0;
  constexpr int BN = BN_, NJ = BN_ / 32, WN = BN_ / 2;
  constexpr int STAGE_BYTES = A_BYTES + BN_ * BK * 2;
  constexpr int GI = 4 + BN_ / 32;
  extern __shared__ __attribute__((aligned(16))) char smem[];
  const int split = p.split_k > 1 ? p.split_k : 1;
  const int lane = threadIdx.x & 63, w = __builtin_amdgcn_readfirstlane(threadIdx.x >> 6);
  const int wm = w >> 1, wn = w & 1;
  const int r = lane & 15, g = lane >> 4;
  int kchunk = (p.K + split - 1) / split;
  kchunk = ((kchunk + BK - 1) / BK) * BK;

  __shared__ long seg_tab[SEG ? 2 : 1][SEG ? 64 : 1];
  if constexpr (SEG) {
    const int nsl = p.K / BK;
    if ((int)threadIdx.x < nsl) {
      const int k = threadIdx.x * BK, sg = k / p.seg_k, within = k - sg * p.seg_k;
      seg_tab[0][threadIdx.x] = p.seg_a_off[sg] + (TA ? (long)within * p.lda : (long)within);
      seg_tab[1][threadIdx.x] = p.seg_b_off ? p.seg_b_off[sg] + (TB ? (long)within : (long)within * p.ldb) : (TB ? (long)k : (long)k * p.ldb);
    }
    __syncthreads();
  }
  struct Tile { const bf16_t* A; const bf16_t* B; long doff; int m0, n0, k_begin, k_end, nfull, tail, ks; const bf16_t* sa[4]; const bf16_t* sb[BN_ / 32]; };
  auto tile_of = [&](int it) {
    Tile T;
    T.nfull = -1;
    const int tpp = gx * gy;
    int tx, ty, tz;
    if constexpr (FIXED) {
      if (it > 0) return T;
      tx = bid % gx; ty = bid / gx; tz = G;
    } else if ((G & 7) == 0) {
      const int x = bid & 7, j = (bid >> 3) + it * (G >> 3);
      if (split > 1 && (gz & 7) == 0) {
        if (j >= (gz >> 3) * tpp) return T;
        tz = x + 8 * (j / tpp);
        const int t = j % tpp;
        tx = t % gx; ty = t / gx;
      } else {
        const int round0 = it * G, R = ntiles - round0, slot = bid >> 3;
        if (R <= 0) return T;
        int t;
        if (R >= G) t = round0 + x * (G >> 3) + slot;
        else {
          const int q = R >> 3, rem = R & 7;
          if (slot >= q + (x < rem ? 1 : 0)) return T;
          t = round0 + (x < rem ? x * (q + 1) : rem * (q + 1) + (x - rem) * q) + slot;
        }
        tx = t % gx; const int rest = t / gx; ty = rest % gy; tz = rest / gy;
      }
    } else {
      if (it > 0) return T;
      const int q = G >> 3, rem = G & 7, xcd = bid & 7, slot = bid >> 3;
      const int t = G >= 16 ? (xcd < rem ? xcd * (q + 1) : rem * (q + 1) + (xcd - rem) * q) + slot : (int)bid;
      tx = t % gx; const int rest = t / gx; ty = rest % gy; tz = rest / gy;
    }
    const int ks = tz % split, bidx = tz / split;
    const int b1 = bidx / p.nb2, b2 = bidx % p.nb2;
    T.A = (const bf16_t*)p.A + b1 * p.sA1 + b2 * p.sA2;
    T.B = (const bf16_t*)p.B + b1 * p.sB1 + b2 * p.sB2;
    T.doff = b1 * p.sD1 + b2 * p.sD2;
    T.m0 = ty * BM;
    if constexpr (SEG) { if (p.row_tiles) T.m0 = min(max(p.row_tiles[ty >> 1], 0) * 256 + (ty & 1) * BM, ((p.M + BM - 1) / BM - 1) * BM); }
    T.n0 = tx * BN;
    T.ks = ks;
    T.k_begin = ks * kchunk;
    T.k_end = min(p.K, T.k_begin + kchunk);
    const int len = max(T.k_end - T.k_begin, 0);
    T.nfull = len / BK;
    T.tail = (len % BK) != 0;
    if (TA) prep_trans<128>(T.sa, T.A, p.lda, T.m0, p.M, T.k_begin, w, lane); else prep_direct<128>(T.sa, T.A, p.lda, T.m0, p.M, T.k_begin, w, lane);
    if (TB) prep_direct<BN_>(T.sb, T.B, p.ldb, T.n0, p.N, T.k_begin, w, lane); else prep_trans<BN_>(T.sb, T.B, p.ldb, T.n0, p.N, T.k_begin, w, lane);
    return T;
  };
  const long stepA = TA ? (long)BK * p.lda : (long)BK, stepB = TB ? (long)BK : (long)BK * p.ldb;
  auto issue = [&](const Tile& T, int slab, int stage) {
    char* sA = smem + stage * STAGE_BYTES;
    char* sB = sA + A_BYTES;
    if constexpr (SEG) {
      issue_from<128>(sA, T.sa, seg_tab[0][slab], w);
      issue_from<BN_>(sB, T.sb, seg_tab[1][slab], w);
    } else {
      issue_from<128>(sA, T.sa, slab * stepA, w);
      issue_from<BN_>(sB, T.sb, slab * stepB, w);
    }
  };

  auto issue_piece = [&](const Tile& T, int slab, int stage, int q) {
    char* sA = smem + stage * STAGE_BYTES;
    char* sB = sA + A_BYTES;
    long dA_, dB_;
    if constexpr (SEG) { dA_ = seg_tab[0][slab]; dB_ = seg_tab[1][slab]; }
    else { dA_ = slab * stepA; dB_ = slab * stepB; }
    if (q < 4) glds16(T.sa[q] + dA_, sA + __builtin_amdgcn_readfirstlane((w * 4 + q) * 1024));
    else glds16(T.sb[q - 4] + dB_, sB + __builtin_amdgcn_readfirstlane((w * (BN_ / 32) + (q - 4)) * 1024));
  };
  Tile cur = tile_of(0);
  if (cur.nfull < 0) return;
  if (cur.nfull > 0) issue(cur, 0, 0);
  if (cur.nfull > 1) issue(cur, 1, 1);
  bool drained = false;

  for (int it = 0;; ++it) {
#ifdef TFASR_GEMM_TIMING
    const long long t_start = __builtin_readcyclecounter();
#endif
    float4_t acc[4][NJ];
#pragma unroll
    for (int i = 0; i < 4; ++i)
#pragma unroll
      for (int j = 0; j < NJ; ++j) acc[i][j] = float4_t{0.f, 0.f, 0.f, 0.f};
    float4_t accb[C_CS ? NJ : 1];
#pragma unroll
    for (int j = 0; j < (C_CS ? NJ : 1); ++j) accb[j] = float4_t{0.f, 0.f, 0.f, 0.f};
    const bool do_cs = C_CS && p.colsum && cur.m0 == 0 && wm == 0;

    constexpr int PF_LPRW = (BN_ / 2) / 8, PF_RPP = 64 / PF_LPRW, PF_NPASS = 16 / PF_RPP;
    constexpr bool PF_Z = (C_DACT || C_MUL) && !GEN && !C_WS;
    [[maybe_unused]] uint4 pf_z[PF_Z ? 4 : 1][PF_Z ? PF_NPASS : 1];
    [[maybe_unused]] bool pf_ok = false;
    auto prefetch_z = [&]() {
      if constexpr (PF_Z) {
        if (!p.accumulate) {
          const int prow = lane / PF_LPRW, col0 = cur.n0 + wn * (BN_ / 2) + (lane % PF_LPRW) * 8;
          pf_ok = ((p.ldd & 7) == 0) && ((cur.doff & 7) == 0) && (col0 + 8 <= p.N) &&
                  p.dact_z && ((((uintptr_t)p.dact_z) & 15) == 0);
          if (pf_ok) {
#pragma unroll
            for (int i = 0; i < 4; ++i)
#pragma unroll
              for (int h = 0; h < PF_NPASS; ++h) {
                const int row = min(cur.m0 + wm * 64 + i * 16 + h * PF_RPP + prow, p.M - 1);
                const long idx0 = cur.doff + (long)row * p.ldd + col0;
                pf_z[i][h] = *reinterpret_cast<const uint4*>((const bf16_t*)p.dact_z + idx0);
              }
          }
        }
      }
    };
    if constexpr (ONE) prefetch_z();
    const int n = cur.nfull;
    __builtin_amdgcn_s_waitcnt(0x0F70);
#ifdef TFASR_GEMM_TIMING
    long long ph[5] = {0, 0, 0, 0, 0};
#define TFASR_TICK(k) { const long long t_ = __builtin_readcyclecounter(); ph[k] += t_ - tp; tp = t_; }
#else
#define TFASR_TICK(k)
#endif
    if constexpr (NST == 3) {
      for (int s = 0; s < n; ++s) {
        const int stage = s % 3;
        if (!(drained && s < 2)) {
          if (s + 1 < n) { if (GI == 8) asm volatile("s_waitcnt vmcnt(8)" ::: "memory"); else asm volatile("s_waitcnt vmcnt(6)" ::: "memory"); }
          else asm volatile("s_waitcnt vmcnt(0)" ::: "memory");
        }
        __builtin_amdgcn_s_barrier();
        if (s + 2 < n) issue(cur, s + 2, (s + 2) % 3);
        mma_slab<TA, TB, BN_, C_CS>(smem + stage * STAGE_BYTES, smem + stage * STAGE_BYTES + A_BYTES, wm, wn, lane, acc, accb, do_cs);
        asm volatile("s_waitcnt lgkmcnt(0)" ::: "memory");
      }
      __builtin_amdgcn_s_barrier();
    } else {
      for (int s = 0; s < n; ++s) {
        const int stage = s & 1;
  #ifdef TFASR_GEMM_TIMING
        long long tp = __builtin_readcyclecounter();
  #endif
        if (!(drained && s < 2)) {
          if (s + 1 < n) { if (GI == 8) asm volatile("s_waitcnt vmcnt(8)" ::: "memory"); else asm volatile("s_waitcnt vmcnt(6)" ::: "memory"); }
          else asm volatile("s_waitcnt vmcnt(0)" ::: "memory");
        }
        TFASR_TICK(0)
        __builtin_amdgcn_s_barrier();
        TFASR_TICK(1)
#ifdef TFASR_FAST_NO_ILV
        mma_slab<TA, TB, BN_, C_CS>(smem + stage * STAGE_BYTES, smem + stage * STAGE_BYTES + A_BYTES, wm, wn, lane, acc, accb, do_cs);
        asm volatile("s_waitcnt lgkmcnt(0)" ::: "memory");
        TFASR_TICK(2)
        __builtin_amdgcn_s_barrier();
        TFASR_TICK(3)
        if (s + 2 < n) issue(cur, s + 2, stage);
        TFASR_TICK(4)
#else
        struct Hook {
          const decltype(issue_piece)& ip; const Tile& T; int slab, stage; bool on;
          __device__ __forceinline__ void reads_done() const {
            asm volatile("s_waitcnt lgkmcnt(0)" ::: "memory");
            __builtin_amdgcn_s_barrier();
          }
          __device__ __forceinline__ void between(int q) const { if (on && q < GI) ip(T, slab, stage, q); }
        };
        const Hook hook{issue_piece, cur, s + 2, stage, s + 2 < n};
        mma_slab<TA, TB, BN_, C_CS, Hook>(smem + stage * STAGE_BYTES, smem + stage * STAGE_BYTES + A_BYTES, wm, wn, lane, acc, accb, do_cs, hook);
        TFASR_TICK(2)
#endif
      }
    }
    if (cur.tail) {
      char* sA = smem;
      char* sB = smem + A_BYTES;
      const int kt = cur.k_begin + n * BK;
      if (TA) tail_trans<128>(sA, cur.A, p.lda, cur.m0, p.M, kt, cur.k_end); else tail_direct<128>(sA, cur.A, p.lda, cur.m0, p.M, kt, cur.k_end);
      if (TB) tail_direct<BN_>(sB, cur.B, p.ldb, cur.n0, p.N, kt, cur.k_end); else tail_trans<BN_>(sB, cur.B, p.ldb, cur.n0, p.N, kt, cur.k_end);
      __syncthreads();
      mma_slab<TA, TB, BN_, C_CS>(sA, sB, wm, wn, lane, acc, accb, do_cs);
      __syncthreads();
    }
    if constexpr (!ONE) prefetch_z();
    Tile nxt;
    if constexpr (ONE) nxt.nfull = -1;
    else {
      nxt = tile_of(it + 1);
      if (nxt.nfull > 0) issue(nxt, 0, 0);
      if (nxt.nfull > 1) issue(nxt, 1, 1);
    }
#ifdef TFASR_GEMM_TIMING
    const long long t_main = __builtin_readcyclecounter();
#endif

    const int m0 = cur.m0, n0 = cur.n0;
    const long doff = cur.doff;
    const bool first_split = (cur.ks == 0);
    bf16_t* Dt = (bf16_t*)p.D + doff;
    float* Df = (float*)p.D + doff;
    const bf16_t* res = p.res ? (const bf16_t*)p.res + doff : nullptr;
    const bf16_t* dz = p.dact_z ? (const bf16_t*)p.dact_z + doff : nullptr;
    bf16_t* prez = p.prez ? (bf16_t*)p.prez + doff : nullptr;
    if constexpr (C_CS) {
      if (do_cs && g == 0) {
#pragma unroll
        for (int j = 0; j < NJ; ++j) {
          const int col = n0 + wn * WN + j * 16 + r;
          if (col < p.N) atomicAdd(p.colsum + col, p.alpha * accb[j][0]);
        }
      }
    }
    if (!C_WS && p.accumulate) {
#pragma unroll
      for (int i = 0; i < 4; ++i)
#pragma unroll
        for (int j = 0; j < NJ; ++j) {
          const int col = n0 + wn * WN + j * 16 + r;
#pragma unroll
          for (int e = 0; e < 4; ++e) {
            const int row = m0 + wm * 64 + i * 16 + g * 4 + e;
            if (col < p.N && row < p.M) {
              float v = p.alpha * acc[i][j][e];
              if (p.bias && first_split) v += p.bias[col];
              atomicAdd(Df + (long)row * p.ldd + col, v);
            }
          }
        }
    } else {
      constexpr int SLD = WN + 4;
      constexpr int LPRW = WN / 8;
      constexpr int RPP = 64 / LPRW;
      constexpr int NPASS = 16 / RPP;
      float* sc = reinterpret_cast<float*>(smem + (ONE ? 0 : NST * STAGE_BYTES)) + w * (RPP * SLD);
      const int prow = lane / LPRW, c8 = (lane % LPRW) * 8;
      const int col0 = n0 + wn * WN + c8;
      const bool vec_ok = C_WS ? ((p.N & 7) == 0) : (((p.ldd & 7) == 0) && ((((uintptr_t)p.D) & 15) == 0) && ((doff & 7) == 0));
      const bool full = vec_ok && (col0 + 8 <= p.N);
      float* wsp = C_WS ? p.ws + (long)cur.ks * p.M * p.N : nullptr;
      float bv[8];
#pragma unroll
      for (int q = 0; q < 8; ++q) bv[q] = 0.f;
      if (p.bias && first_split && col0 < p.N) {
// ... 196 lines not shown
      strips(std::integral_constant<int, 1>{});
      strips(std::integral_constant<int, 2>{});
      strips(std::integral_constant<int, 3>{});
      if constexpr (C_BNS) {
        static_assert(LPRW == 4 || LPRW == 8, "rows of 4 or 8 lanes");
        float* out = p.bns_out + (size_t)(bid % (p.bns_copies > 0 ? p.bns_copies : 1)) * 2 * bnc;
#pragma unroll
        for (int q = 0; q < 8; ++q) {
          float a0 = bs0[q], a1 = bs1[q];
          a0 += dpp_mov<0x128>(a0); a1 += dpp_mov<0x128>(a1);
          if constexpr (LPRW == 4) { a0 += dpp_mov<0x124>(a0); a1 += dpp_mov<0x124>(a1); }
          a0 = xor32_sum(xor16_sum(a0)); a1 = xor32_sum(xor16_sum(a1));
          if (lane < LPRW && col0 + 8 <= p.N) { atomicAdd(out + bcol + q, a0); atomicAdd(out + bnc + bcol + q, a1); }
        }
      }
    }
#ifdef TFASR_GEMM_TIMING
    if (threadIdx.x == 0 && it == 0) {
      const long long t_end = __builtin_readcyclecounter();
      long long* o = g_gemm_timing + 4L * bid;
      o[0] = t_start; o[1] = 0; o[2] = t_main - t_start; o[3] = t_end - t_start;
    }
    if (threadIdx.x == 0 && it == 1) {
      const long long t_end = __builtin_readcyclecounter();
      long long* o = g_gemm_timing + 4L * 32768 + 2L * bid;
      o[0] = t_main - t_start; o[1] = t_end - t_start;
    }
    if (threadIdx.x == 0 && it == 0) {
      long long* o = g_gemm_timing + 6L * 32768 + 5L * bid;
      for (int k = 0; k < 5; ++k) o[k] = ph[k];
    }
#endif
    if (nxt.nfull < 0) break;
    __builtin_amdgcn_s_waitcnt(0x0F70);
    asm volatile("" ::: "memory");
    drained = true;
    cur = nxt;
  }
}

template <bool TA, bool TB, int BN_, int EPI>
__global__ __launch_bounds__(256, 2) void gemm_fast_kernel(const tfasr_gemm_args p, const int gx, const int gy, const int gz, const int ntiles) {
  gemm_fast_body<TA, TB, BN_, EPI>(p, gx, gy, gz, ntiles, (int)blockIdx.x, (int)gridDim.x);
}
template <bool TA, bool TB, int EPI>
__global__ __launch_bounds__(256, 3) void gemm_fast_one_kernel(const tfasr_gemm_args p, const int gx, const int gy, const int gz, const int ntiles) {
  gemm_fast_body<TA, TB, 64, EPI, 2, false, false, true>(p, gx, gy, gz, ntiles, (int)blockIdx.x, (int)gridDim.x);
}
template <bool TA, bool TB>
__global__ __launch_bounds__(256, 2) void gemm_seg_kernel(const tfasr_gemm_args p, const int gx, const int gy, const int gz, const int ntiles) {
  gemm_fast_body<TA, TB, 128, 0, 2, false, true>(p, gx, gy, gz, ntiles, (int)blockIdx.x, (int)gridDim.x);
}

constexpr int GROUP_MAX = 10;
constexpr int GROUP_UNITS = 20;
struct GroupArgs {
  tfasr_gemm_args p[GROUP_MAX];
  int gx[GROUP_MAX], gy[GROUP_MAX];
  short uq[8][GROUP_UNITS], uks[8][GROUP_UNITS];
  int j0[8][GROUP_UNITS + 1];
  int nunit[8];
};
template <int EPI, int NST, int BN_>
__global__ __launch_bounds__(256, 2) void wgrad_group_kernel(const GroupArgs ga) {
  const int x = blockIdx.x & 7, j = blockIdx.x >> 3;
  const int nu = ga.nunit[x];
  int u = -1;
  for (int i = 0; i < nu; ++i)
    if (j >= ga.j0[x][i] && j < ga.j0[x][i + 1]) u = i;
  u = __builtin_amdgcn_readfirstlane(u);
  if (u < 0) return;
  const int q = ga.uq[x][u], ks = ga.uks[x][u], t = j - ga.j0[x][u];
  const tfasr_gemm_args* pp = ga.p + q;
  gemm_fast_body<true, false, BN_, EPI, NST, true>(*pp, ga.gx[q], ga.gy[q], 1, ga.gx[q] * ga.gy[q], t, ks);
}

__global__ __launch_bounds__(256) void splitk_reduce_kernel(const float* __restrict__ ws, float* __restrict__ D, int M, int N, int ldd, int split) {
  const long mn = (long)M * N;
  if ((N & 3) == 0 && (ldd & 3) == 0 && ((((uintptr_t)D) & 15) == 0)) {
    const int n4 = N >> 2;
    for (long i = (long)blockIdx.x * blockDim.x + threadIdx.x; i < mn / 4; i += (long)gridDim.x * blockDim.x) {
      float4 acc = *reinterpret_cast<const float4*>(ws + 4 * i);
      for (int s2 = 1; s2 < split; ++s2) {
        const float4 t = *reinterpret_cast<const float4*>(ws + s2 * mn + 4 * i);
        acc.x += t.x; acc.y += t.y; acc.z += t.z; acc.w += t.w;
      }
      const long m = i / n4;
      float4* d = reinterpret_cast<float4*>(D + m * ldd + 4 * (i - m * n4));
      float4 o = *d;
      o.x += acc.x; o.y += acc.y; o.z += acc.z; o.w += acc.w;
      *d = o;
    }
  } else {
    for (long i = (long)blockIdx.x * blockDim.x + threadIdx.x; i < mn; i += (long)gridDim.x * blockDim.x) {
      float acc = 0.f;
      for (int s2 = 0; s2 < split; ++s2) acc += ws[s2 * mn + i];
      const long m = i / N;
      D[m * ldd + (i - m * N)] += acc;
    }
  }
}

int num_cus();

int num_cus() {
  static int n = 0;
  if (n == 0) {
    int dev = 0, v = 0;
    if (hipGetDevice(&dev) == hipSuccess && hipDeviceGetAttribute(&v, hipDeviceAttributeMultiprocessorCount, dev) == hipSuccess && v > 0) n = v;
    else n = 256;
  }
  return n;
}

template <bool TA, bool TB, int BN_, int EPI>
int launch_epi(const tfasr_gemm_args& a, dim3 tiles, hipStream_t stream) {
  const long ntiles = (long)tiles.x * tiles.y * tiles.z;
  static const int per_cu = 2;
  const int slots = per_cu * num_cus();
  if constexpr (BN_ == 64 && (EPI & (E_WS | E_CSUM | E_LSE)) == 0) {
    static const bool one_off = false;
    static const long one_max = (1L << 30);
    if (!one_off && a.split_k <= 1 && ntiles > slots && ntiles <= one_max * num_cus()) {
      constexpr int SMEM1 = 2 * (A_BYTES + 64 * BK * 2);
      TFASR_KLAUNCH((gemm_fast_one_kernel<TA, TB, EPI>), dim3((unsigned)ntiles), dim3(256), SMEM1, stream, a, (int)tiles.x, (int)tiles.y, (int)tiles.z, (int)ntiles);
      TFASR_CHECK_LAUNCH();
      return TFASR_STATUS_SUCCESS;
    }
  }
  int G = (int)(ntiles < slots ? ntiles : slots);
  if (ntiles >= slots) G &= ~7;
  constexpr int SMEM = 2 * (A_BYTES + BN_ * BK * 2) + 4 * (64 / (BN_ / 16)) * (BN_ / 2 + 4) * 4;
  TFASR_KLAUNCH((gemm_fast_kernel<TA, TB, BN_, EPI>), dim3(G), dim3(256), SMEM, stream, a, (int)tiles.x, (int)tiles.y, (int)tiles.z, (int)ntiles);
  TFASR_CHECK_LAUNCH();
  return TFASR_STATUS_SUCCESS;
}

#include "gemm_big.h"
#include "ffn_fused.h"
#include "dense_ln.h"

template <bool TA, bool TB>
int launch_one(const tfasr_gemm_args& a, hipStream_t stream) {
  const int split = a.split_k > 1 ? a.split_k : 1;
  static const bool bn64_off = false;
  const long t128 = (long)((a.N + 127) / 128) * ((a.M + BM - 1) / BM) * a.nb1 * a.nb2 * split;
  static const long bn64_thr = (1L << 40);
  const long bn64_lim = (split <= 1 && !a.accumulate && !a.colsum && std::min(a.K, a.N) <= 256) ? bn64_thr : std::min(bn64_thr, (long)num_cus());
  const bool narrow = !a.lse_part && !a.seg_a_off && (a.N <= 64 || (!bn64_off && t128 <= bn64_lim && a.N > 64 && !(a.accumulate && a.ws)));
  const int bn = narrow ? 64 : 128;
  dim3 grid((a.N + bn - 1) / bn, (a.M + BM - 1) / BM, a.nb1 * a.nb2 * split);
  if ((long)grid.x * grid.y * grid.z > 0x7fffffffL) return TFASR_STATUS_INVALID_VALUE;
  int need = 0;
  bool generic = false;
  if (!a.accumulate) {
    if (a.out_f32) generic = true;
    if (a.act != TFASR_ACT_NONE || a.prez) { if (a.act == TFASR_ACT_SWISH) need |= E_ACT; else generic = true; }
    if (a.dact_z) { if (a.dact == TFASR_ACT_SWISH) need |= E_DACT; else if (a.dact == TFASR_ACT_FACTOR) need |= E_MUL; else generic = true; }
    if (a.drop_p > 0.f) need |= E_DROP;
    if (a.res) need |= E_RES;
  }
  if (a.bns_out) {
    if constexpr (!TA && TB) {
      if (narrow && !generic && need == 0 && !a.accumulate && !a.bias && split == 1 && a.nb1 * a.nb2 == 1 && a.bns_x && a.bns_fin && (a.N & 7) == 0 && (a.ldd & 7) == 0 &&
          (a.bns_c == 0 || (a.bns_c > 0 && (a.bns_c & 7) == 0 && a.N % a.bns_c == 0)) &&
          (((uintptr_t)a.D | (uintptr_t)a.bns_x) & 15) == 0 && !a.colsum && !a.lse_part && !a.seg_a_off && !a.rgrad_coef)
        return launch_epi<TA, TB, 64, E_BNS>(a, grid, stream);
    }
    return TFASR_STATUS_UNSUPPORTED;
  }
  if constexpr (!TA) {
    const bool tanh_out = !a.accumulate && a.dact_z && a.dact == TFASR_ACT_TANH_OUT;
    const bool other = a.out_f32 || a.act != TFASR_ACT_NONE || a.prez || (a.dact_z && !tanh_out);
    const int st = launch_big<TB>(a, other, need, tanh_out, stream);
    if (st != TFASR_STATUS_UNSUPPORTED) return st;
  }
  if (a.rgrad_coef || !a.D) return TFASR_STATUS_UNSUPPORTED;
  if (a.accumulate && split > 1 && a.nb1 * a.nb2 == 1 && a.ws && a.ws_elems >= (long)split * a.M * a.N && !narrow && !a.colsum) {
    const int st = launch_epi<TA, TB, 128, E_WS>(a, grid, stream);
    if (st != TFASR_STATUS_SUCCESS) return st;
    const long work = ((long)a.M * a.N + 3) / 4;
    const int rg = (int)(work / 256 + 1 < 2048 ? work / 256 + 1 : 2048);
    TFASR_KLAUNCH(splitk_reduce_kernel, dim3(rg), dim3(256), 0, stream, (const float*)a.ws, (float*)a.D, a.M, a.N, a.ldd, split);
    TFASR_CHECK_LAUNCH();
    return TFASR_STATUS_SUCCESS;
  }
  if (a.colsum) {
    if constexpr (TA && !TB) {
      if (a.accumulate && a.N > 64) return narrow ? launch_epi<TA, TB, 64, E_CSUM>(a, grid, stream) : launch_epi<TA, TB, 128, E_CSUM>(a, grid, stream);
    }
    return TFASR_STATUS_UNSUPPORTED;
  }
  if (narrow) {
    if (!generic && need == 0) return launch_epi<TA, TB, 64, 0>(a, grid, stream);
    if constexpr (!TA && !TB) {
      if (!generic && need == E_RES) return launch_epi<TA, TB, 64, E_RES>(a, grid, stream);
      if (!generic && need == (E_RES | E_DROP)) return launch_epi<TA, TB, 64, E_RES | E_DROP>(a, grid, stream);
// ... 7 lines not shown
        if (need == E_DACT) return launch_epi<TA, TB, 64, E_DACT>(a, grid, stream);
        if (need == (E_DACT | E_DROP)) return launch_epi<TA, TB, 64, E_DACT | E_DROP>(a, grid, stream);
        if (need == E_MUL) return launch_epi<TA, TB, 64, E_MUL>(a, grid, stream);
      }
    }
    return launch_epi<TA, TB, 64, E_GEN>(a, grid, stream);
  }
  if (a.seg_a_off) {
    if constexpr (!TA) {
      if (!generic && need == 0 && !a.accumulate && split == 1 && a.nb1 * a.nb2 == 1 && a.seg_k > 0 && (a.seg_k % BK) == 0 && (a.K % a.seg_k) == 0 &&
          a.K / BK <= 64 && !a.lse_part) {
        dim3 g128((a.N + 127) / 128, a.row_tiles ? 2 * a.n_row_tiles : (a.M + BM - 1) / BM, 1);
        const long ntiles = (long)g128.x * g128.y;
        const int slots = 2 * num_cus();
        int G = (int)(ntiles < slots ? ntiles : slots);
        if (ntiles >= slots) G &= ~7;
        constexpr int SMEM = 2 * (A_BYTES + 128 * BK * 2) + 4 * (64 / (128 / 16)) * (128 / 2 + 4) * 4;
        TFASR_KLAUNCH((gemm_seg_kernel<TA, TB>), dim3(G), dim3(256), SMEM, stream, a, (int)g128.x, (int)g128.y, 1, (int)ntiles);
        TFASR_CHECK_LAUNCH();
        return TFASR_STATUS_SUCCESS;
      }
    }
    return TFASR_STATUS_UNSUPPORTED;
  }
  if (a.lse_part) {
    if constexpr (!TA && !TB) {
      if (!generic && need == 0 && !a.accumulate && a.nb1 * a.nb2 == 1 && a.row_label && a.pick && a.lse_parts == ((a.N + 127) / 128) * 2)
        return launch_epi<TA, TB, 128, E_LSE>(a, grid, stream);
    }
    return TFASR_STATUS_UNSUPPORTED;
  }
  if (!generic) {
    if (need == 0) return launch_epi<TA, TB, 128, 0>(a, grid, stream);
    if constexpr (!TA && !TB) {
      if (need == E_RES) return launch_epi<TA, TB, 128, E_RES>(a, grid, stream);
      if (need == (E_RES | E_DROP)) return launch_epi<TA, TB, 128, E_RES | E_DROP>(a, grid, stream);
      if (need == E_ACT) return launch_epi<TA, TB, 128, E_ACT>(a, grid, stream);
      if (need == (E_ACT | E_DROP)) return launch_epi<TA, TB, 128, E_ACT | E_DROP>(a, grid, stream);
    }
    if constexpr (!TA && TB) {
      if (need == E_DACT) return launch_epi<TA, TB, 128, E_DACT>(a, grid, stream);
      if (need == (E_DACT | E_DROP)) return launch_epi<TA, TB, 128, E_DACT | E_DROP>(a, grid, stream);
      if (need == E_MUL) return launch_epi<TA, TB, 128, E_MUL>(a, grid, stream);
    }
  }
  return launch_epi<TA, TB, 128, E_GEN>(a, grid, stream);
}

inline bool al16(const void* p) { return (((uintptr_t)p) & 15) == 0; }

bool group_eligible(const tfasr_gemm_args& a) {
  return a.dtype == TFASR_BF16 && a.trans_a && !a.trans_b && a.accumulate && a.out_f32 && a.nb1 * a.nb2 <= 1 && !a.ws && !a.bias && !a.res &&
         !a.dact_z && !a.prez && a.act == TFASR_ACT_NONE && a.drop_p == 0.f && al16(a.A) && al16(a.B) && !(a.lda & 7) && !(a.ldb & 7) &&
         ((a.M + 7) & ~7) <= a.lda && ((a.N + 7) & ~7) <= a.ldb && a.K >= 8 && a.N > 64 && a.M > 0;
}

}

int g_tfasr_group_beside = 0;

int tfasr_gemm_group_fast_try(const tfasr_gemm_args* a, int n, hipStream_t stream) {
  if (n < 2 || n > GROUP_MAX) return TFASR_STATUS_UNSUPPORTED;
  for (int i = 0; i < n; ++i)
    if (!group_eligible(a[i])) return TFASR_STATUS_UNSUPPORTED;
  GroupArgs ga;
  memset(&ga, 0, sizeof(ga));
  long total = 0;
  static const int bn = 128;
  for (int i = 0; i < n; ++i) {
    ga.gx[i] = (a[i].N + bn - 1) / bn;
    ga.gy[i] = (a[i].M + BM - 1) / BM;
    total += (long)ga.gx[i] * ga.gy[i];
  }
  static const long env_slots = 0;
  long kmax = 0;
  for (int i = 0; i < n; ++i) kmax = a[i].K > kmax ? a[i].K : kmax;
  const long slots = env_slots > 0 ? env_slots : ((g_tfasr_group_beside || kmax >= 131072) ? num_cus() * 5L / 4 : 2L * num_cus());
  long split = slots / (total > 0 ? total : 1);
  if (split < 1) split = 1;
  {
    static const bool dbg = false;
    static int dbg_n = 0;
    if (dbg && dbg_n < 6) { fprintf(stderr, "[group] n %d tiles %ld beside %d slots %ld split %ld\n", n, total, g_tfasr_group_beside, slots, split); ++dbg_n; }
  }
  struct U { int q, ks, tiles; };
  U units[GROUP_MAX * 64];
  int nu = 0;
  for (int i = 0; i < n; ++i) {
    long sp = split;
    if (a[i].K / 512 < sp) sp = a[i].K / 512;
    if (sp < 1) sp = 1;
    if (sp > 64) sp = 64;
    ga.p[i] = a[i];
    ga.p[i].split_k = (int)sp;
    ga.p[i].nb1 = ga.p[i].nb2 = 1;
    for (int k2 = 0; k2 < (int)sp; ++k2) units[nu++] = U{i, k2, ga.gx[i] * ga.gy[i]};
  }
  for (int i = 1; i < nu; ++i) {
    const U v = units[i];
    int j = i - 1;
    while (j >= 0 && units[j].tiles < v.tiles) { units[j + 1] = units[j]; --j; }
    units[j + 1] = v;
  }
  int load[8] = {0, 0, 0, 0, 0, 0, 0, 0};
  for (int i = 0; i < nu; ++i) {
    int best = 0;
    for (int x = 1; x < 8; ++x)
      if (load[x] < load[best]) best = x;
    const int c = ga.nunit[best];
    if (c >= GROUP_UNITS) return TFASR_STATUS_UNSUPPORTED;
    ga.uq[best][c] = (short)units[i].q;
    ga.uks[best][c] = (short)units[i].ks;
    ga.j0[best][c] = load[best];
    load[best] += units[i].tiles;
    ga.j0[best][c + 1] = load[best];
    ga.nunit[best] = c + 1;
  }
  int maxload = 0;
  for (int x = 0; x < 8; ++x)
    if (load[x] > maxload) maxload = load[x];
  static const int nst = 2;
  if (bn == 64) {
    constexpr int STAGE = A_BYTES + 64 * BK * 2;
    if (nst == 3) TFASR_KLAUNCH((wgrad_group_kernel<E_CSUM, 3, 64>), dim3(8 * maxload), dim3(256), 3 * STAGE, stream, ga);
    else TFASR_KLAUNCH((wgrad_group_kernel<E_CSUM, 2, 64>), dim3(8 * maxload), dim3(256), 2 * STAGE, stream, ga);
  } else {
    constexpr int STAGE = A_BYTES + 128 * BK * 2;
    TFASR_KLAUNCH((wgrad_group_kernel<E_CSUM, 2, 128>), dim3(8 * maxload), dim3(256), 2 * STAGE, stream, ga);
  }
  TFASR_CHECK_LAUNCH();
  return TFASR_STATUS_SUCCESS;
}

int tfasr_gemm_fast_try(const tfasr_gemm_args& a, hipStream_t stream) {
  if (a.dtype != TFASR_BF16) return TFASR_STATUS_UNSUPPORTED;
  if (!al16(a.A) || !al16(a.B) || (a.lda & 7) || (a.ldb & 7)) return TFASR_STATUS_UNSUPPORTED;
  if ((a.sA1 & 7) || (a.sA2 & 7) || (a.sB1 & 7) || (a.sB2 & 7)) return TFASR_STATUS_UNSUPPORTED;
  if (a.trans_a && ((a.M + 7) & ~7) > a.lda) return TFASR_STATUS_UNSUPPORTED;
  if (!a.trans_b && ((a.N + 7) & ~7) > a.ldb) return TFASR_STATUS_UNSUPPORTED;
  if (a.K < 8) return TFASR_STATUS_UNSUPPORTED;
  if (a.trans_a) return a.trans_b ? launch_one<true, true>(a, stream) : launch_one<true, false>(a, stream);
  return a.trans_b ? launch_one<false, true>(a, stream) : launch_one<false, false>(a, stream);
}

extern "C" int tfasr_ffn_fused_fwd2(const void* x, const float* gamma, const float* beta, const void* W1, const float* b1, const void* W2,
                                    const float* b2, void* y, void* ln, float* mean, float* rstd, void* z, int z_factor, void* h, long rows, int d, int F,
                                    float ln_eps, float res_factor, float drop_p, long drop_seed1, long drop_seed2, int dtype, void* stream);
extern "C" int tfasr_ffn_fused_fwd(const void* x, const float* gamma, const float* beta, const void* W1, const float* b1, const void* W2,
                                   const float* b2, void* y, void* ln, float* mean, float* rstd, void* z, void* h, long rows, int d, int F,
                                   float ln_eps, float res_factor, float drop_p, long drop_seed1, long drop_seed2, int dtype, void* stream) {
  return tfasr_ffn_fused_fwd2(x, gamma, beta, W1, b1, W2, b2, y, ln, mean, rstd, z, 0, h, rows, d, F, ln_eps, res_factor, drop_p, drop_seed1, drop_seed2, dtype, stream);
}
extern "C" int tfasr_ffn_fused_fwd2(const void* x, const float* gamma, const float* beta, const void* W1, const float* b1, const void* W2,
                                    const float* b2, void* y, void* ln, float* mean, float* rstd, void* z, int z_factor, void* h, long rows, int d, int F,
                                    float ln_eps, float res_factor, float drop_p, long drop_seed1, long drop_seed2, int dtype, void* stream) {
  if (!x || !gamma || !beta || !W1 || !b1 || !W2 || !b2 || !y || !ln || !mean || !rstd || rows <= 0 || d <= 0 || F <= 0) return TFASR_STATUS_INVALID_VALUE;
  if (!(drop_p >= 0.f && drop_p < 1.f)) return TFASR_STATUS_INVALID_VALUE;
  static const bool off = getenv("TFASR_FFN_FUSED") && getenv("TFASR_FFN_FUSED")[0] == '0';
  if (off || dtype != TFASR_BF16 || d != 256 || (F % 64) != 0 || F > 1024 || F < 128 || rows * (long)F >= (1L << 32)) return TFASR_STATUS_UNSUPPORTED;
  const uintptr_t al = (uintptr_t)x | (uintptr_t)W1 | (uintptr_t)W2 | (uintptr_t)y | (uintptr_t)ln | (uintptr_t)z | (uintptr_t)h | (uintptr_t)gamma | (uintptr_t)beta;
  if (al & 15) return TFASR_STATUS_UNSUPPORTED;
  FfnArgs a;
  a.x = (const bf16_t*)x; a.gamma = gamma; a.beta = beta; a.W1 = (const bf16_t*)W1; a.b1 = b1; a.W2 = (const bf16_t*)W2; a.b2 = b2;
  a.y = (bf16_t*)y; a.ln = (bf16_t*)ln; a.mean = mean; a.rstd = rstd; a.z = (bf16_t*)z; a.h = (bf16_t*)h;
  a.rows = rows; a.F = F; a.eps = ln_eps; a.res = res_factor; a.drop_p = drop_p; a.seed1 = drop_seed1; a.seed2 = drop_seed2;
  a.zfactor = z_factor ? 1 : 0;
  a.dbg = nullptr;
#ifdef TFASR_FFN_TIMING
  static long long* dbg_buf = nullptr;
  if (!dbg_buf && hipMalloc((void**)&dbg_buf, 64) != hipSuccess) dbg_buf = nullptr;
  a.dbg = dbg_buf;
#endif
  const int st = launch_ffn_fused_fwd(a, (hipStream_t)stream);
#ifdef TFASR_FFN_TIMING
  if (dbg_buf) {
    long long h[8];
    if (hipStreamSynchronize((hipStream_t)stream) == hipSuccess && hipMemcpy(h, dbg_buf, 64, hipMemcpyDeviceToHost) == hipSuccess)
      fprintf(stderr, "[ffn_timing] prologue %lld | per-kernel sums: wait+barrier %lld dma-issue %lld gemm1 %lld z->lds %lld rowpass %lld gemm2 %lld | epilogue %lld\n",
              h[0], h[1], h[2], h[3], h[4], h[5], h[6], h[7]);
  }
#endif
// ... 38 lines not shown
```

tensorflowasr_amd/kernels.py:

```python
import ctypes
import os

import torch

from . import _lib
from ._lib import ACT_FACTOR, ACT_NONE, ACT_SIGMOID, ACT_SWISH, ACT_TANH, ACT_TANH_OUT, TFASR_BF16, TFASR_F32, GemmArgs, check

_WS_CACHE = {}
_SPLITK_WS = False


def _dt(t):
    if t.dtype == torch.float32:
        return TFASR_F32
    if t.dtype == torch.bfloat16:
        return TFASR_BF16
    raise TypeError(f"unsupported activation dtype {t.dtype}")


def _p(t):
    if t is None:
        return None
    if not t.is_cuda:
        raise _lib.TfasrError("tensorflowasr_amd ops need HIP device tensors (no CPU fallback on the product path)")
# ... 168 lines not shown
                                                    B, T, U + 1, V, blank, _p(frames), _p(label_lp), _p(score), _p(ws), ws.numel(), _stream()),
                 "rnnt_align_stats")
    return frames, label_lp, score


def ctc_align(logits, labels, label_len, logit_len, blank=0, normalized=False):
    assert logits.dim() == 3 and labels.dim() == 2 and labels.dtype == torch.int32 and labels.is_contiguous()
    B, T, V = logits.shape
    U = labels.shape[1]
    assert labels.shape[0] == B and label_len.dtype == torch.int32 and logit_len.dtype == torch.int32
    dev = logits.device
    start = torch.empty(B, U, dtype=torch.int32, device=dev)
    end = torch.empty(B, U, dtype=torch.int32, device=dev)
    label_lp = torch.empty(B, U, dtype=torch.float32, device=dev)
    score = torch.empty(B, dtype=torch.float32, device=dev)
    ws = workspace(ctc_align_workspace_size(B, T, U, V), dev, "align")
    _align_check(_lib.load().tfasr_ctc_align(_p(logits), _p(labels) if U else None, _p(label_len), _p(logit_len), B, T, U, V, blank, _dt(logits),
                                             1 if normalized else 0, _p(start) if U else None, _p(end) if U else None, _p(label_lp) if U else None,
                                             _p(score), _p(ws), ws.numel(), _stream()), "ctc_align")
    return start, end, label_lp, score


def _edit_check(st, what):
    if st == _lib.STATUS_UNSUPPORTED:
        raise _lib.TfasrUnsupported(f"{what}: a sequence width above TFASR_EDIT_MAX_LEN (see include/tfasr_hip.h)")
    check(st, what)


def edit_distance_workspace_size(P, N, M):
    n = ctypes.c_size_t(0)
    _edit_check(_lib.load().tfasr_edit_distance_workspace_size(P, N, M, ctypes.byref(n)), "edit_distance_workspace_size")
    return n.value


def edit_distance(hyp, ref, hyp_len=None, ref_len=None, skip_id=-1):
    for t in (hyp, ref, hyp_len, ref_len):
        if t is not None and not t.is_cuda:
            raise _lib.TfasrError("tensorflowasr_amd ops need HIP device tensors (no CPU fallback on the product path)")
    assert hyp.dim() == 2 and ref.dim() == 2 and hyp.shape[0] == ref.shape[0] and hyp.dtype == torch.int32 and ref.dtype == torch.int32
    P, N, M = hyp.shape[0], hyp.shape[1], ref.shape[1]
    for ln in (hyp_len, ref_len):
        assert ln is None or (ln.dtype == torch.int32 and ln.shape == (P,))
    counts = torch.empty(P, 5, dtype=torch.int32, device=hyp.device)
    if P == 0:
        return counts
    ws = workspace(edit_distance_workspace_size(P, N, M), hyp.device, "edit")
    _edit_check(_lib.load().tfasr_edit_distance(_p(hyp) if N else _p(counts), _p(hyp_len), _p(ref) if M else _p(counts), _p(ref_len), P, N, M,
                                                 int(skip_id), _p(counts), _p(ws), ws.numel(), _stream()), "edit_distance")
    return counts


def gemm(A, B, out, M, N, K, lda, ldb, ldd, trans_a=False, trans_b=False, bias=None, res=None, dact_z=None,
         prez=None, alpha=1.0, beta=1.0, act=ACT_NONE, dact=ACT_NONE, nb1=1, nb2=1, sA=(0, 0), sB=(0, 0), sD=(0, 0),
         accumulate=False, split_k=1, drop_p=0.0, drop_seed=0, colsum=None, lse=None, seg=None, rgrad=None, bns=None, row_tiles=None):
    a = _gemm_args(A, B, out, M, N, K, lda, ldb, ldd, trans_a, trans_b, bias, res, dact_z, prez, alpha, beta, act, dact, nb1, nb2, sA, sB, sD,
                   accumulate, split_k, drop_p, drop_seed, colsum)
    if rgrad is not None:
        coef, row_label = rgrad
        assert coef.dtype == torch.float32 and coef.is_contiguous() and row_label.dtype == torch.int32
        a.rgrad_coef, a.row_label = coef.data_ptr(), row_label.data_ptr()
    if seg is not None:
        a.seg_a_off, a.seg_b_off, a.seg_k = seg[0].data_ptr(), (seg[1].data_ptr() if seg[1] is not None else None), int(seg[2])
        assert seg[0].dtype == torch.int64 and seg[0].is_cuda
    if row_tiles is not None:
        assert seg is not None and row_tiles.dtype == torch.int32 and row_tiles.is_cuda and row_tiles.is_contiguous()
        a.row_tiles, a.n_row_tiles = row_tiles.data_ptr(), row_tiles.numel()
    if bns is not None:
        bx, bfin, bout = bns[:3]
        bc = int(bns[3]) if len(bns) > 3 else N
        assert bfin.dtype == torch.float32 and bout.dtype == torch.float32 and bout.is_contiguous()
        a.bns_x, a.bns_fin, a.bns_out, a.bns_copies = bx.data_ptr(), bfin.data_ptr(), bout.data_ptr(), bout.numel() // (2 * bc)
        a.bns_c = 0 if bc == N else bc
    if lse is not None:
        part, row_label, pick = lse
        assert part.dtype == torch.float32 and pick.dtype == torch.float32 and row_label.dtype == torch.int32
        a.lse_part, a.lse_parts, a.row_label, a.pick = part.data_ptr(), part.shape[1], row_label.data_ptr(), pick.data_ptr()
    st = _lib.load().tfasr_gemm(ctypes.byref(a), _stream())
    if (lse is not None or seg is not None or rgrad is not None or bns is not None) and st == _lib.STATUS_UNSUPPORTED:
        raise _lib.TfasrUnsupported("gemm: fused row statistics / K-segments / gradient epilogue are not available for this product")
    check(st, "gemm")
    return out


def gemm_group(calls):
    arr = (GemmArgs * len(calls))()
    for i, kw in enumerate(calls):
        arr[i] = _gemm_args(**kw)
    check(_lib.load().tfasr_gemm_group(arr, len(calls), _stream()), "gemm_group")


def _gemm_args(A, B, out, M, N, K, lda, ldb, ldd, trans_a=False, trans_b=False, bias=None, res=None, dact_z=None,
               prez=None, alpha=1.0, beta=1.0, act=ACT_NONE, dact=ACT_NONE, nb1=1, nb2=1, sA=(0, 0), sB=(0, 0), sD=(0, 0),
               accumulate=False, split_k=1, drop_p=0.0, drop_seed=0, colsum=None):
    a = GemmArgs()
    a.A, a.B, a.D = A.data_ptr(), B.data_ptr(), (out.data_ptr() if out is not None else None)
    a.bias = bias.data_ptr() if bias is not None else None
    a.res = res.data_ptr() if res is not None else None
    a.dact_z = dact_z.data_ptr() if dact_z is not None else None
    a.prez = prez.data_ptr() if prez is not None else None
    a.M, a.N, a.K = M, N, K
    a.lda, a.ldb, a.ldd = lda, ldb, ldd
    a.trans_a, a.trans_b = int(trans_a), int(trans_b)
    a.nb1, a.nb2 = nb1, nb2
    a.sA1, a.sA2, a.sB1, a.sB2, a.sD1, a.sD2 = sA[0], sA[1], sB[0], sB[1], sD[0], sD[1]
    a.alpha, a.beta = alpha, beta
    a.act, a.dact = act, dact
    a.dtype = _dt(A)
    assert B.dtype == A.dtype and A.is_cuda and B.is_cuda and (out is None or out.is_cuda)
    a.out_f32 = int(out is not None and out.dtype == torch.float32)
    a.accumulate = int(accumulate)
    a.split_k = split_k
    a.drop_p, a.drop_seed = drop_p, drop_seed
    a.colsum = colsum.data_ptr() if colsum is not None else None
    if accumulate:
        assert out.dtype == torch.float32
        if _SPLITK_WS and split_k > 1 and nb1 * nb2 == 1:
            ws = workspace(4 * split_k * M * N, out.device, "splitk_%d" % (_raw_stream(torch.cuda.current_device()) if _raw_stream else 0))
            a.ws, a.ws_elems = ws.data_ptr(), ws.numel() // 4
    return a


def matmul(A, B, trans_a=False, trans_b=False, out=None, out_dtype=None, **kw):
    M, K = (A.shape[1], A.shape[0]) if trans_a else (A.shape[0], A.shape[1])
    N = B.shape[0] if trans_b else B.shape[1]
    if out is None:
        out = torch.empty(M, N, dtype=out_dtype or A.dtype, device=A.device)
    return gemm(A, B, out, M, N, K, A.stride(0), B.stride(0), out.stride(0), trans_a, trans_b, **kw)


def _L():
    return _lib.load()


def layernorm_fwd(x, gamma, beta, eps=1e-3, save_stats=True):
    rows, C = x.numel() // x.shape[-1], x.shape[-1]
    y = torch.empty_like(x)
    mean = torch.empty(rows, dtype=torch.float32, device=x.device) if save_stats else None
    rstd = torch.empty(rows, dtype=torch.float32, device=x.device) if save_stats else None
    check(_L().tfasr_layernorm_fwd(_p(x), _p(gamma), _p(beta), _p(y), _p(mean), _p(rstd), rows, C, eps, _dt(x), _stream()), "layernorm_fwd")
    return y, mean, rstd


def ffn_fused_fwd(x, gamma, beta, W1, b1, W2, b2, res_factor, drop_p=0.0, seed1=0, seed2=0, save_z=True, eps=1e-3, z_factor=False):
    rows, d = x.shape
    F = W1.shape[1]
    y, ln = torch.empty_like(x), torch.empty_like(x)
    mean = torch.empty(rows, dtype=torch.float32, device=x.device)
    rstd = torch.empty(rows, dtype=torch.float32, device=x.device)
    z = torch.empty(rows, F, dtype=x.dtype, device=x.device) if save_z else None
    h = torch.empty(rows, F, dtype=x.dtype, device=x.device)
    st = _L().tfasr_ffn_fused_fwd2(_p(x), _p(gamma), _p(beta), _p(W1), _p(b1), _p(W2), _p(b2), _p(y), _p(ln), _p(mean), _p(rstd), _pv(z), int(bool(z_factor)),
                                   _p(h), rows, d, F, eps, float(res_factor), float(drop_p), int(seed1), int(seed2), _dt(x), _stream())
    if st == _lib.STATUS_UNSUPPORTED:
        return None
    check(st, "ffn_fused_fwd")
    return y, ln, mean, rstd, z, h


def ln_dense_fwd(x, gamma, beta, W, b, eps=1e-3):
    rows, d = x.shape
    N = W.shape[1]
    out = torch.empty(rows, N, dtype=x.dtype, device=x.device)
    ln = torch.empty_like(x)
    mean = torch.empty(rows, dtype=torch.float32, device=x.device)
    rstd = torch.empty(rows, dtype=torch.float32, device=x.device)
    st = _L().tfasr_ln_dense_fwd(_p(x), _p(gamma), _p(beta), _p(W), _p(b), _p(out), _p(ln), _p(mean), _p(rstd), rows, d, N, eps, _dt(x), _stream())
    if st == _lib.STATUS_UNSUPPORTED:
        return None
    check(st, "ln_dense_fwd")
# ... 497 lines not shown
    B, T0, F0 = x.shape[:3]
    C = dy.shape[-1]
    check(_L().tfasr_conv1_bwd_weight(_p(x), _p(dy), _p(dw), _p(db), B, T0, F0, C, _dt(x), _stream()), "conv1_bwd_weight")


def conv1_fwd_s2d(x, w, bias, y):
    B, T0, F0 = x.shape[:3]
    check(_L().tfasr_conv1_fwd_s2d(_p(x), _p(w), _p(bias), _p(y), B, T0, F0, w.shape[-1], _dt(x), _stream()), "conv1_fwd_s2d")
    return y


def conv1_bwd_weight_s2d(x, dy, dw, db, C):
    B, T0, F0 = x.shape[:3]
    check(_L().tfasr_conv1_bwd_weight_s2d(_p(x), _p(dy), _p(dw), _p(db), B, T0, F0, C, _dt(x), _stream()), "conv1_bwd_weight_s2d")


def conv1_stats(x, w, bias, stats):
    B, T0, F0 = x.shape[:3]
    check(_L().tfasr_conv1_stats(_p(x), _p(w), _p(bias), _p(stats), B, T0, F0, w.shape[-1], _dt(x), _stream()), "conv1_stats")


def conv1_bn_apply_s2d(x, w, bias, fin, y):
    B, T0, F0 = x.shape[:3]
    check(_L().tfasr_conv1_bn_apply_s2d(_p(x), _p(w), _p(bias), _p(fin), _p(y), B, T0, F0, w.shape[-1], _dt(x), _stream()), "conv1_bn_apply")
    return y


def conv1_bn_bwd_stats_s2d(x, w, bias, fin, dy, bstats):
    B, T0, F0 = x.shape[:3]
    check(_L().tfasr_conv1_bn_bwd_stats_s2d(_p(x), _p(w), _p(bias), _p(fin), _p(dy), _p(bstats), B, T0, F0, w.shape[-1], _dt(x), _stream()),
          "conv1_bn_bwd_stats")


def conv1_bn_bwd_apply_s2d(x, w, bias, fin, bstats, count, dy, dw, db):
    B, T0, F0 = x.shape[:3]
    check(_L().tfasr_conv1_bn_bwd_apply_s2d(_p(x), _p(w), _p(bias), _p(fin), _p(bstats), float(count), _p(dy), _p(dw), _p(db), B, T0, F0,
                                            w.shape[-1], _dt(x), _stream()), "conv1_bn_bwd_apply")


CONV1_GRAM_DOUBLES = 768


def conv1_gram(x, gram):
    B, T0, F0 = x.shape[:3]
    assert gram.dtype == torch.float64 and gram.numel() >= CONV1_GRAM_DOUBLES
    check(_L().tfasr_conv1_gram(_p(x), _p(gram), B, T0, F0, _dt(x), _stream()), "conv1_gram")
    return gram


def conv1_stats_from_gram(gram, w, bias, stats):
    check(_L().tfasr_conv1_stats_from_gram(_p(gram), _p(w), _p(bias), _p(stats), w.shape[-1], _stream()), "conv1_stats_from_gram")


def conv1_bn_bwd_onepass_s2d(x, w, bias, fin, dy, bstats, pbuf):
    B, T0, F0 = x.shape[:3]
    check(_L().tfasr_conv1_bn_bwd_onepass_s2d(_p(x), _p(w), _p(bias), _p(fin), _p(dy), _p(bstats), _p(pbuf), B, T0, F0, w.shape[-1], _dt(x),
                                              _stream()), "conv1_bn_bwd_onepass")


def conv1_bn_bwd_finalize(gram, w, bias, fin, bstats, count, pbuf, dw, db):
    check(_L().tfasr_conv1_bn_bwd_finalize(_p(gram), _p(w), _p(bias), _p(fin), _p(bstats), float(count), _p(pbuf), _p(dw), _p(db), w.shape[-1],
                                           _stream()), "conv1_bn_bwd_finalize")


def halo_zero(x, B, T2, F2, W):
    check(_L().tfasr_halo_zero(_p(x), B, T2, F2, W, _dt(x), _stream()), "halo_zero")
    return x


def s2d_edge_zero(x, B, T1, F1, C):
    check(_L().tfasr_s2d_edge_zero(_p(x), B, T1, F1, C, _dt(x), _stream()), "s2d_edge_zero")


def s2d_tail_fill(x, tiles, rep_tt, B, T2, F2, C):
    assert tiles.dtype == torch.int32 and rep_tt.dtype == torch.int32 and tiles.is_cuda and rep_tt.is_cuda and rep_tt.numel() == B
    st = _L().tfasr_s2d_tail_fill(_p(x), _p(tiles), tiles.numel(), _p(rep_tt), B, T2, F2, C, _dt(x), _stream())
    if st == _lib.STATUS_UNSUPPORTED:
        raise _lib.TfasrUnsupported("s2d_tail_fill: bf16 tensors with C % 8 == 0 only")
    check(st, "s2d_tail_fill")
    return x


def im2col_3x3s2(x, col=None):
    B, T1, F1, C = x.shape
    T2, F2 = (T1 + 1) // 2, (F1 + 1) // 2
    if col is None:
        col = torch.empty(B * T2 * F2, 9 * C, dtype=x.dtype, device=x.device)
    check(_L().tfasr_im2col_3x3s2(_p(x), _p(col), B, T1, F1, C, _dt(x), _stream()), "im2col")
    return col


def col2im_3x3s2(dcol, B, T1, F1, C):
    dx = torch.empty(B, T1, F1, C, dtype=dcol.dtype, device=dcol.device)
    check(_L().tfasr_col2im_3x3s2(_p(dcol), _p(dx), B, T1, F1, C, _dt(dcol), _stream()), "col2im")
    return dx


def logmel(signal, window, melw, band, frame_step, nfft, preemph, eps, out_dtype):
    B, N = signal.shape
    T0 = -(-N // frame_step)
    F = melw.shape[1]
    out = torch.empty(B, T0, F, dtype=out_dtype, device=signal.device)
    assert signal.dtype == torch.float32
    check(_L().tfasr_logmel(_p(signal), B, N, preemph, _p(window), window.numel(), frame_step, nfft, _p(melw), _p(band), F,
                            eps, _p(out), T0, _dt(out), _stream()), "logmel")
    return out


def decode_prepare(encj, nframes, frame_idx, tok_idx, active, ecur, max_tokens, mode):
    B, T, J = encj.shape
    check(_L().tfasr_decode_prepare(_p(encj), _p(nframes), _p(frame_idx), _p(tok_idx), _p(active), _p(ecur), B, T, J, max_tokens,
                                    mode, _dt(encj), _stream()), "decode_prepare")


def decode_pack(emb, lstm_k, lstm_rk, wjp, wv):
    V, E = emb.shape
    P = lstm_rk.shape[0]
    J = wv.shape[0]
    n = int(_L().tfasr_decode_pack_floats(E, P, J, V))
    if n == 0:
        return None
    packed = torch.empty(n, dtype=torch.float32, device=lstm_k.device)
    st = _L().tfasr_decode_pack(_p(emb), _p(lstm_k), _p(lstm_rk), _p(wjp), _p(wv), _p(packed), E, P, J, V, _stream())
    if st == _lib.STATUS_UNSUPPORTED:
        return None
    check(st, "decode_pack")
    return packed


def decode_step(emb, lstm_k, lstm_rk, lstm_b, ln_g, ln_b, wjp, bjp, wv, bv, encj, nframes, frame_idx, tok_idx, prev_tok, h, c, active, h_new, c_new,
                z, logits, max_tokens, mode, ln_eps=1e-3, packed=None):
    B, T, J = encj.shape
# ... 940 lines not shown
```

Measured before the change: 4.843 audio-hours/sec.

## Fold padded subsampling tail in backward and skip padded K-blocks and rows

In the subsampling conv backward, gradient rows in each utterance's padded tail are summed into three representative rows. The sum is split as hi/mid/lo bf16 parts so it stays exact under linearity, and the other tail rows are zeroed. The conv1 weight-grad grouped GEMM then iterates only over a table of real K-blocks, the data-grad GEMM computes only real row tiles, and the conv0 BN backward one-pass kernel visits only listed rows. This removes wasted work on padding frames in the front-end backward, at the cost of an extra fold kernel, atomics, host-built tables, and a reliance on the padded input rows being identical.

```diff
diff --git a/include/tfasr_hip.h b/include/tfasr_hip.h
--- a/include/tfasr_hip.h
+++ b/include/tfasr_hip.h
@@ -84,6 +84,7 @@
   const void* bns_x; const float* bns_fin; float* bns_out; int bns_copies;
   int bns_c;
   const int32_t* row_tiles; int n_row_tiles;
+  const int32_t* k_tiles; int n_k_tiles;
 } tfasr_gemm_args;
 
 int tfasr_gemm(const tfasr_gemm_args* args, void* stream);
@@ -301,12 +302,15 @@
 int tfasr_conv1_stats_from_gram(const double* gram, const float* w, const float* bias, float* stats, int C, void* stream);
 int tfasr_conv1_bn_bwd_onepass_s2d(const void* x, const float* w, const float* bias, const float* fin, const void* dy, float* bstats,
                                    float* pbuf, int B, int T0, int F0, int C, int dtype, void* stream);
+int tfasr_conv1_bn_bwd_onepass_s2d_rows(const void* x, const float* w, const float* bias, const float* fin, const void* dy, float* bstats,
+                                        float* pbuf, int B, int T0, int F0, int C, int dtype, const int32_t* row_list, int n_rows, void* stream);
 int tfasr_conv1_bn_bwd_finalize(const double* gram, const float* w, const float* bias, const float* fin, const float* bstats, float count,
                                 const float* pbuf, float* dw, float* db, int C, void* stream);
 int tfasr_halo_zero(void* x, int B, int T2, int F2, int W, int dtype, void* stream);
 int tfasr_s2d_edge_zero(void* x, int B, int T1, int F1, int C, int dtype, void* stream);
 int tfasr_s2d_tail_fill(void* x, const int32_t* tiles, int n_tiles, const int32_t* rep_tt, int B, int T2, int F2, int C, int dtype,
                         void* stream);
+int tfasr_s2d_tail_fold(void* x, const int32_t* r_tt, float* scratch, int B, int T2, int F2, int C, int dtype, void* stream);
 int tfasr_im2col_3x3s2(const void* x, void* col, int B, int T1, int F1, int C, int dtype, void* stream);
 int tfasr_col2im_3x3s2(const void* dcol, void* dx, int B, int T1, int F1, int C, int dtype, void* stream);
 
diff --git a/tensorflowasr_amd/_lib.py b/tensorflowasr_amd/_lib.py
--- a/tensorflowasr_amd/_lib.py
+++ b/tensorflowasr_amd/_lib.py
@@ -31,6 +31,7 @@
         ("rgrad_coef", c_void_p),
         ("bns_x", c_void_p), ("bns_fin", c_void_p), ("bns_out", c_void_p), ("bns_copies", c_int), ("bns_c", c_int),
         ("row_tiles", c_void_p), ("n_row_tiles", c_int),
+        ("k_tiles", c_void_p), ("n_k_tiles", c_int),
     ]
 
 
diff --git a/tensorflowasr_amd/conformer.py b/tensorflowasr_amd/conformer.py
--- a/tensorflowasr_amd/conformer.py
+++ b/tensorflowasr_amd/conformer.py
@@ -58,6 +58,7 @@
         self._bn_stats_copies = 8
         self._conv1_gram = True
         self._sub_tail_once = os.environ.get("TFASR_SUB_TAIL", "1") != "0"
+        self._sub_tail_bwd = os.environ.get("TFASR_SUB_TAIL_BWD", "1") != "0"
         self._front_tail = None
         self._rng = np.random.default_rng([seed + 1000, int(self.dp.rank)])
         prio = -1
@@ -192,6 +193,11 @@
         has = rep + 1 <= T2
         rep = np.where(has, rep, 1)
         end = np.where(has, rep + 1, T2 + 1)
+        real = cls._real_blocks(end, B, T2, F2)
+        return np.flatnonzero(real), np.flatnonzero(~real), rep
+
+    @staticmethod
+    def _real_blocks(end, B, T2, F2):
         nblk = -(-(B * (T2 + 1) * (F2 + 1)) // 256)
         base = np.arange(B, dtype=np.int64) * (T2 + 1)
         lo = (base + 1) * (F2 + 1) // 256
@@ -199,8 +205,18 @@
         mark = np.zeros(nblk + 1, np.int64)
         np.add.at(mark, lo, 1)
         np.add.at(mark, hi + 1, -1)
-        real = np.cumsum(mark[:nblk]) > 0
-        return np.flatnonzero(real), np.flatnonzero(~real), rep
+        return np.cumsum(mark[:nblk]) > 0
+
+    @classmethod
+    def _tail_bwd_geometry(cls, tf, B, T0, T2, F2):
+        T1 = (T0 + 1) // 2
+        r = cls._tail_rows(tf, T0)["o"]
+        fold = r + 3 <= T2
+        end = np.where(fold, r + 3, T2 + 1)
+        real = cls._real_blocks(end, B, T2, F2)
+        n1 = np.where(fold, np.minimum(T1, 2 * (r + 2)), T1)
+        rows = np.concatenate([b * T1 + np.arange(n1[b], dtype=np.int64) for b in range(B)])
+        return np.flatnonzero(real), np.flatnonzero(~real), np.where(fold, r, T2 + 1), rows
 
     def _tail_tables(self, tf, B, T0, T2, F2):
         key = ("tail", tf, T0, F2)
@@ -210,8 +226,13 @@
         comp, skip, rep = self._tail_blocks(tf, B, T0, T2, F2)
         out = None
         if skip.size * 16 >= comp.size + skip.size:
-            dev = self._h2d(np.concatenate([comp, skip, rep]).astype(np.int32))
-            out = (dev[:comp.size], dev[comp.size:comp.size + skip.size], dev[comp.size + skip.size:])
+            parts = [comp, skip, rep]
+            bcomp, bskip, r, rows = self._tail_bwd_geometry(tf, B, T0, T2, F2)
+            if bskip.size * 16 >= bcomp.size + bskip.size:
+                parts += [bcomp, r, rows]
+            dev = self._h2d(np.concatenate(parts).astype(np.int32))
+            out = tuple(torch.split(dev, [p.size for p in parts]))
+            out = out[:3] + (out[3:] if len(out) > 3 else None,)
         old = [k for k in self._consts if isinstance(k, tuple) and k[:1] == ("tail",)]
         for k in old[:max(0, len(old) - 7)]:
             del self._consts[k]
@@ -341,7 +362,7 @@
         w0, b0 = ps.p("enc/sub/conv0/w"), ps.p("enc/sub/conv0/b")
         fin0 = torch.empty(4 * C, dtype=torch.float32, device=self.device)
         nm = "enc/sub/bn0"
-        gram = None
+        gram, tail_bwd = None, None
         if training:
             stats = self._zeros_f32(2 * C + 1)[:2 * C + 1]
             if self._conv1_gram:
@@ -369,8 +390,12 @@
                        bias=ps.p("enc/sub/conv1/b") if i == 0 else None, accumulate=i > 0)
         else:
             tail, ft, self._front_tail = None, self._front_tail, None
-            if self._sub_tail_once and ft is not None and ft[0] is feats and ft[1] is not None and len(ft[1]) == B:
+            if (self._sub_tail_once or self._sub_tail_bwd) and ft is not None and ft[0] is feats and ft[1] is not None and len(ft[1]) == B:
                 tail = self._tail_tables(ft[1], B, T0, T2, F2)
+            if tail is not None and training and self._sub_tail_bwd and gram is not None:
+                tail_bwd = tail[3]
+            if not self._sub_tail_once:
+                tail = None
             if tail is not None:
                 try:
                     K.gemm(a1, W, o, rows, C, 9 * C, 4 * C, C, C, bias=ps.p("enc/sub/conv1/b"), seg=fwd_a, row_tiles=tail[0])
@@ -392,7 +417,7 @@
         elen = [-(-(-(-n // 2)) // 2) for n in flen]
         if ctx is not None:
             ctx["sub"] = dict(s2d=True, feats=feats, bn0=bn0, a1=a1, a1_full=a1_full, o=o, bn1=bn1, a2=a2,
-                              dims=(B, T0, F0, T1, F1, T2, F2), drop=drop)
+                              dims=(B, T0, F0, T1, F1, T2, F2), drop=drop, tail_bwd=tail_bwd)
         return x0, T2, elen
 
     def _subsampling_bwd_s2d(self, dx0, ctx):
@@ -430,12 +455,19 @@
             K.bn_apply_bwd(s["o"], da2, fin1, bst, count1, ACT_SWISH, dx=do, dgamma=ps.g("enc/sub/bn1/g"), dbeta=ps.g("enc/sub/bn1/b"),
                            grad_scale=1.0 / self.dp.world, copies=ncp)
         K.halo_zero(do, B, T2, F2, C)
+        tb = s.get("tail_bwd") if self._sub_tail_bwd else None
+        if tb is not None and not (self.dtype == torch.bfloat16 and C % 64 == 0 and s["bn0"][2] is not None and do.data_ptr() % 16 == 0):
+            tb = None
+        if tb is not None:
+            K.s2d_tail_fold(do, tb[1], self._zeros_f32(B * (F2 + 1) * C)[:B * (F2 + 1) * C], B, T2, F2, C)
+        kt, nk = (None, rows) if tb is None else (tb[0], 256 * tb[0].numel())
         a1_full, base = s["a1_full"], slack * 4 * C
         gW = ps.g2d("enc/sub/conv1/w")
         calls = []
         for i in range(9):
             calls.append(dict(A=a1_full[base + shift[i] * 4 * C + blk[i] * C:], B=do, out=gW[i * C:(i + 1) * C], M=C, N=C, K=rows, lda=4 * C, ldb=C,
-                              ldd=C, trans_a=True, accumulate=True, split_k=_split_k(C, C, rows), colsum=ps.g("enc/sub/conv1/b") if i == 0 else None))
+                              ldd=C, trans_a=True, accumulate=True, split_k=_split_k(C, C, nk), colsum=ps.g("enc/sub/conv1/b") if i == 0 else None,
+                              k_tiles=kt))
         K.gemm_group(calls)
         W = ps.w2d("enc/sub/conv1/w")
         _, da1 = self._salloc(rows, 4 * C, 0)
@@ -447,13 +479,14 @@
                 for j, i in enumerate(segs):
                     K.gemm(do_full[dobase - shift[i] * C:], W[i * C:(i + 1) * C], out, rows, C, C, C, C, 4 * C, trans_b=True, accumulate=j > 0)
             else:
-                K.gemm(do, W, out, rows, C, len(segs) * C, C, C, 4 * C, trans_b=True, seg=(a_off, b_off, C // (a_off.numel() // len(segs))))
+                K.gemm(do, W, out, rows, C, len(segs) * C, C, C, 4 * C, trans_b=True, seg=(a_off, b_off, C // (a_off.numel() // len(segs))),
+                       row_tiles=None if tb is None else tb[0])
         fin0, count0, gram = s["bn0"]
         w0, b0 = ps.p("enc/sub/conv0/w"), ps.p("enc/sub/conv0/b")
         if gram is not None:
             zz = self._zeros_f32(12 * C)
             bstats, pbuf = zz[:2 * C], zz[2 * C:12 * C]
-            K.conv1_bn_bwd_onepass_s2d(s["feats"], w0, b0, fin0, da1, bstats, pbuf)
+            K.conv1_bn_bwd_onepass_s2d(s["feats"], w0, b0, fin0, da1, bstats, pbuf, row_list=None if tb is None else tb[2])
             self.dp.allreduce_stats_(bstats)
             K.conv1_bn_bwd_finalize(gram, w0, b0, fin0, bstats, count0, pbuf, ps.g("enc/sub/conv0/w"), ps.g("enc/sub/conv0/b"))
         else:
diff --git a/tensorflowasr_amd/csrc/conv2d.hip b/tensorflowasr_amd/csrc/conv2d.hip
--- a/tensorflowasr_amd/csrc/conv2d.hip
+++ b/tensorflowasr_amd/csrc/conv2d.hip
@@ -273,7 +273,8 @@
 __global__ __launch_bounds__(256) void conv1_bn_kernel(const T* __restrict__ x, const float* __restrict__ w, const float* __restrict__ bias,
                                                        const float* __restrict__ fin, const float* __restrict__ bstats, float inv_count,
                                                        T* __restrict__ y, const T* __restrict__ dy, float* __restrict__ out0,
-                                                       float* __restrict__ out1, int B, int T0, int F0, int T1, int F1, int C) {
+                                                       float* __restrict__ out1, int B, int T0, int F0, int T1, int F1, int C,
+                                                       const int32_t* __restrict__ row_list, int n_list) {
   extern __shared__ float sm[];
   float* xs = sm;
   float* red = sm + 3 * (F0 + 2);
@@ -312,8 +313,10 @@
   for (int q = 0; q < NQ; ++q)
 #pragma unroll
     for (int k = 0; k < CP2; ++k) acc2[q][k] = c1f2_t{0.f, 0.f};
-  const int nrows = B * T1;
-  for (int row = blockIdx.x; row < nrows; row += gridDim.x) {
+  const bool listed = MODE == 4 && row_list != nullptr;
+  const int nrows = listed ? n_list : B * T1;
+  for (int it = blockIdx.x; it < nrows; it += gridDim.x) {
+    const int row = listed ? min(max(row_list[it], 0), B * T1 - 1) : it;
     const int b = row / T1, t = row - b * T1;
     __syncthreads();
     for (int i = threadIdx.x; i < 3 * (F0 + 2); i += 256) {
@@ -582,6 +585,57 @@
   }
 }
 
+
+constexpr int FOLD_TT = 32;
+__global__ __launch_bounds__(256) void s2d_tail_sum_kernel(bf16_t* __restrict__ x, const int32_t* __restrict__ r_tt, float* __restrict__ scratch,
+                                                           int T2, int F2, int C, int zr) {
+  const int b = blockIdx.y, r = r_tt[b];
+  if (r < 1 || r + 3 > T2) return;
+  const int t0 = max(r, 1 + (int)blockIdx.x * FOLD_TT), t1 = min(T2 + 1, 1 + ((int)blockIdx.x + 1) * FOLD_TT);
+  if (t0 >= t1) return;
+  const int per_t = (F2 + 1) * C;
+  const float z[8] = {0, 0, 0, 0, 0, 0, 0, 0};
+  for (int i = threadIdx.x * 8; i < per_t; i += 256 * 8) {
+    float acc[8] = {0, 0, 0, 0, 0, 0, 0, 0};
+    for (int tt = t0; tt < t1; ++tt) {
+      bf16_t* p = x + ((long)b * (T2 + 1) + tt) * per_t + i;
+      float v[8];
+      ld8(p, v);
+#pragma unroll
+      for (int k = 0; k < 8; ++k) acc[k] += v[k];
+      if (tt >= r + 3 && (tt < r + 3 + zr || tt > T2 - zr)) st8(p, z);
+    }
+    float* s = scratch + (long)b * per_t + i;
+#pragma unroll
+    for (int k = 0; k < 8; ++k) atomicAdd(s + k, acc[k]);
+  }
+}
+__global__ __launch_bounds__(256) void s2d_tail_put_kernel(bf16_t* __restrict__ x, const int32_t* __restrict__ r_tt, const float* __restrict__ scratch,
+                                                           int B, int T2, int F2, int C) {
+  const int per_t = (F2 + 1) * C;
+  const long n = (long)B * per_t / 8;
+  for (long j = (long)blockIdx.x * blockDim.x + threadIdx.x; j < n; j += (long)gridDim.x * blockDim.x) {
+    const int b = (int)(j * 8 / per_t), i = (int)(j * 8 - (long)b * per_t);
+    const int r = r_tt[b];
+    if (r < 1 || r + 3 > T2) continue;
+    float s[8], hi[8], mid[8];
+    ld8(scratch + (long)b * per_t + i, s);
+    bf16_t* p = x + ((long)b * (T2 + 1) + r) * per_t + i;
+#pragma unroll
+    for (int k = 0; k < 8; k += 2) {
+      const uint32_t h = pack2_bf16(s[k], s[k + 1]);
+      hi[k] = __uint_as_float(h << 16); hi[k + 1] = __uint_as_float(h & 0xffff0000u);
+      s[k] -= hi[k]; s[k + 1] -= hi[k + 1];
+      const uint32_t m = pack2_bf16(s[k], s[k + 1]);
+      mid[k] = __uint_as_float(m << 16); mid[k + 1] = __uint_as_float(m & 0xffff0000u);
+      s[k] -= mid[k]; s[k + 1] -= mid[k + 1];
+    }
+    st8(p, hi);
+    st8(p + per_t, mid);
+    st8(p + 2 * per_t, s);
+  }
+}
+
 }
 
 #define DISPATCH_T(dtype, CALL_F32, CALL_BF16) \
@@ -654,8 +708,10 @@
 
 template <int MODE>
 static int conv1_bn_launch(const void* x, const float* w, const float* bias, const float* fin, const float* bstats, float count, void* y,
-                           const void* dy, float* out0, float* out1, int B, int T0, int F0, int C, int dtype, void* stream_) {
+                           const void* dy, float* out0, float* out1, int B, int T0, int F0, int C, int dtype, void* stream_,
+                           const int32_t* row_list = nullptr, int n_list = 0) {
   if (!x || !w || B <= 0 || T0 <= 0 || F0 <= 0 || C <= 0 || C > 256 || (C % 8)) return TFASR_STATUS_INVALID_VALUE;
+  if (row_list && (MODE != 4 || n_list <= 0 || n_list > (long)B * ((T0 + 1) / 2))) return TFASR_STATUS_INVALID_VALUE;
   constexpr int CPT = MODE >= 2 ? 4 : 8;
   constexpr int NQL = MODE == 3 ? 10 : (MODE == 4 ? 11 : 2);
   const int T1 = (T0 + 1) / 2, F1 = (F0 + 1) / 2;
@@ -675,14 +731,14 @@
     res_blocks[di] = (e == hipSuccess && per > 0 && cus > 0) ? per * cus : 768;
     res_smem[di] = smem_q;
   }
-  const int grid = std::min(B * T1, MODE == 1 ? 8192 : std::max(64, env_grid ? env_grid : res_blocks[di]));
+  const int grid = std::min(row_list ? n_list : B * T1, MODE == 1 ? 8192 : std::max(64, env_grid ? env_grid : res_blocks[di]));
   const size_t smem = (size_t)(3 * (F0 + 2) + NQL * C) * sizeof(float);
   const float inv = count > 0.f ? 1.f / count : 0.f;
   DISPATCH_T(dtype,
              TFASR_KLAUNCH((conv1_bn_kernel<float, MODE, CPT>), dim3(grid), dim3(256), smem, s, (const float*)x, w, bias, fin, bstats, inv, (float*)y,
-                                (const float*)dy, out0, out1, B, T0, F0, T1, F1, C),
+                                (const float*)dy, out0, out1, B, T0, F0, T1, F1, C, row_list, n_list),
              TFASR_KLAUNCH((conv1_bn_kernel<bf16_t, MODE, CPT>), dim3(grid), dim3(256), smem, s, (const bf16_t*)x, w, bias, fin, bstats, inv, (bf16_t*)y,
-                                (const bf16_t*)dy, out0, out1, B, T0, F0, T1, F1, C));
+                                (const bf16_t*)dy, out0, out1, B, T0, F0, T1, F1, C, row_list, n_list));
   TFASR_CHECK_LAUNCH();
   return TFASR_STATUS_SUCCESS;
 }
@@ -727,10 +783,15 @@
   TFASR_CHECK_LAUNCH();
   return TFASR_STATUS_SUCCESS;
 }
+extern "C" int tfasr_conv1_bn_bwd_onepass_s2d_rows(const void* x, const float* w, const float* bias, const float* fin, const void* dy, float* bstats,
+                                                   float* pbuf, int B, int T0, int F0, int C, int dtype, const int32_t* row_list, int n_rows,
+                                                   void* stream_) {
+  if (!fin || !dy || !bstats || !pbuf) return TFASR_STATUS_INVALID_VALUE;
+  return conv1_bn_launch<4>(x, w, bias, fin, nullptr, 0.f, nullptr, dy, bstats, pbuf, B, T0, F0, C, dtype, stream_, row_list, row_list ? n_rows : 0);
+}
 extern "C" int tfasr_conv1_bn_bwd_onepass_s2d(const void* x, const float* w, const float* bias, const float* fin, const void* dy, float* bstats,
                                               float* pbuf, int B, int T0, int F0, int C, int dtype, void* stream_) {
-  if (!fin || !dy || !bstats || !pbuf) return TFASR_STATUS_INVALID_VALUE;
-  return conv1_bn_launch<4>(x, w, bias, fin, nullptr, 0.f, nullptr, dy, bstats, pbuf, B, T0, F0, C, dtype, stream_);
+  return tfasr_conv1_bn_bwd_onepass_s2d_rows(x, w, bias, fin, dy, bstats, pbuf, B, T0, F0, C, dtype, nullptr, 0, stream_);
 }
 extern "C" int tfasr_conv1_bn_bwd_finalize(const double* gram, const float* w, const float* bias, const float* fin, const float* bstats,
                                            float count, const float* pbuf, float* dw, float* db, int C, void* stream_) {
@@ -775,6 +836,18 @@
   return TFASR_STATUS_SUCCESS;
 }
 
+extern "C" int tfasr_s2d_tail_fold(void* x, const int32_t* r_tt, float* scratch, int B, int T2, int F2, int C, int dtype, void* stream_) {
+  if (!x || !r_tt || !scratch || B <= 0 || T2 <= 0 || F2 <= 0 || C <= 0) return TFASR_STATUS_INVALID_VALUE;
+  if (dtype != TFASR_BF16 || C % 8 || (((uintptr_t)x) & 15) || (((uintptr_t)scratch) & 15) || B > 65535) return TFASR_STATUS_UNSUPPORTED;
+  hipStream_t s = (hipStream_t)stream_;
+  const int zr = (255 + F2 + 2 + F2) / (F2 + 1) + 1;
+  TFASR_KLAUNCH(s2d_tail_sum_kernel, dim3((T2 + FOLD_TT - 1) / FOLD_TT, B), dim3(256), 0, s, (bf16_t*)x, r_tt, scratch, T2, F2, C, zr);
+  TFASR_CHECK_LAUNCH();
+  TFASR_KLAUNCH(s2d_tail_put_kernel, dim3(flat_grid((long)B * (F2 + 1) * C / 8)), dim3(256), 0, s, (bf16_t*)x, r_tt, scratch, B, T2, F2, C);
+  TFASR_CHECK_LAUNCH();
+  return TFASR_STATUS_SUCCESS;
+}
+
 extern "C" int tfasr_im2col_3x3s2(const void* x, void* col, int B, int T1, int F1, int C, int dtype, void* stream_) {
   if (!x || !col || B <= 0 || T1 <= 0 || F1 <= 0 || C <= 0 || C % 8) return TFASR_STATUS_INVALID_VALUE;
   const int T2 = (T1 + 1) / 2, F2 = (F1 + 1) / 2;
diff --git a/tensorflowasr_amd/csrc/gemm.hip b/tensorflowasr_amd/csrc/gemm.hip
--- a/tensorflowasr_amd/csrc/gemm.hip
+++ b/tensorflowasr_amd/csrc/gemm.hip
@@ -416,11 +416,16 @@
     if (a.n_row_tiles <= 0 || a.n_row_tiles > (a.M + 255) / 256) return TFASR_STATUS_INVALID_VALUE;
     if (!a.seg_a_off || a.trans_a || a.accumulate || a.split_k > 1 || a.nb1 * a.nb2 != 1 || a.dtype != TFASR_BF16) return TFASR_STATUS_UNSUPPORTED;
   }
+  if (a.k_tiles) {
+    if (a.n_k_tiles <= 0 || a.n_k_tiles > (a.K + 255) / 256) return TFASR_STATUS_INVALID_VALUE;
+    if (!a.trans_a || a.trans_b || !a.accumulate || a.nb1 * a.nb2 != 1 || a.dtype != TFASR_BF16 || a.seg_a_off || a.row_tiles || a.ws) return TFASR_STATUS_UNSUPPORTED;
+  }
   hipStream_t stream = (hipStream_t)stream_;
   if (a.dtype == TFASR_BF16 && use_fast_path()) {
     const int st = tfasr_gemm_fast_try(a, stream);
     if (st != TFASR_STATUS_UNSUPPORTED) return st;
   }
+  if (a.k_tiles) return TFASR_STATUS_UNSUPPORTED;
   if (a.lse_part || a.rgrad_coef || a.bns_out) return TFASR_STATUS_UNSUPPORTED;
   if (a.seg_a_off) return TFASR_STATUS_UNSUPPORTED;
   if (a.colsum) {
diff --git a/tensorflowasr_amd/csrc/gemm_fast.hip b/tensorflowasr_amd/csrc/gemm_fast.hip
--- a/tensorflowasr_amd/csrc/gemm_fast.hip
+++ b/tensorflowasr_amd/csrc/gemm_fast.hip
@@ -219,7 +219,7 @@
 
 enum : int { E_ACT = 1 , E_DACT = 2 , E_DROP = 4, E_RES = 8, E_WS = 16 , E_CSUM = 32 , E_LSE = 64 , E_RGRAD = 128 , E_GEN = 256, E_BNS = 512 , E_MUL = 1024  };
 
-template <bool TA, bool TB, int BN_, int EPI, int NST = 2, bool FIXED = false, bool SEG = false, bool ONE = false>
+template <bool TA, bool TB, int BN_, int EPI, int NST = 2, bool FIXED = false, bool SEG = false, bool ONE = false, bool KT = false>
 __device__ __forceinline__ void gemm_fast_body(const tfasr_gemm_args& p, const int gx, const int gy, const int gz, const int ntiles, const int bid, const int G) {
   constexpr bool GEN = (EPI & E_GEN) != 0;
   constexpr bool C_ACT = GEN || (EPI & E_ACT), C_DACT = GEN || (EPI & E_DACT), C_DROP = GEN || (EPI & E_DROP), C_RES = GEN || (EPI & E_RES);
@@ -236,8 +236,18 @@
   const int lane = threadIdx.x & 63, w = __builtin_amdgcn_readfirstlane(threadIdx.x >> 6);
   const int wm = w >> 1, wn = w & 1;
   const int r = lane & 15, g = lane >> 4;
-  int kchunk = (p.K + split - 1) / split;
+  int Keff = p.K;
+  if constexpr (KT) {
+    const int nkt = p.n_k_tiles, last = min(max(p.k_tiles[nkt - 1], 0), (p.K - 1) / 256);
+    Keff = (nkt - 1) * 256 + min(256, p.K - last * 256);
+  }
+  int kchunk = (Keff + split - 1) / split;
   kchunk = ((kchunk + BK - 1) / BK) * BK;
+  auto kt_row = [&](int c) -> long {
+    const int blk = min(max(p.k_tiles[min(c >> 2, p.n_k_tiles - 1)], 0), (p.K - 1) / 256);
+    return (long)blk * 256 + (c & 3) * BK;
+  };
+  long kt_dA = 0, kt_dB = 0;
 
   __shared__ long seg_tab[SEG ? 2 : 1][SEG ? 64 : 1];
   if constexpr (SEG) {
@@ -293,13 +303,21 @@
     T.n0 = tx * BN;
     T.ks = ks;
     T.k_begin = ks * kchunk;
-    T.k_end = min(p.K, T.k_begin + kchunk);
+    T.k_end = min(Keff, T.k_begin + kchunk);
     const int len = max(T.k_end - T.k_begin, 0);
     T.nfull = len / BK;
     T.tail = (len % BK) != 0;
-    if (TA) prep_trans<128>(T.sa, T.A, p.lda, T.m0, p.M, T.k_begin, w, lane); else prep_direct<128>(T.sa, T.A, p.lda, T.m0, p.M, T.k_begin, w, lane);
-    if (TB) prep_direct<BN_>(T.sb, T.B, p.ldb, T.n0, p.N, T.k_begin, w, lane); else prep_trans<BN_>(T.sb, T.B, p.ldb, T.n0, p.N, T.k_begin, w, lane);
+    const int kp = KT ? 0 : T.k_begin;
+    if (TA) prep_trans<128>(T.sa, T.A, p.lda, T.m0, p.M, kp, w, lane); else prep_direct<128>(T.sa, T.A, p.lda, T.m0, p.M, kp, w, lane);
+    if (TB) prep_direct<BN_>(T.sb, T.B, p.ldb, T.n0, p.N, kp, w, lane); else prep_trans<BN_>(T.sb, T.B, p.ldb, T.n0, p.N, kp, w, lane);
     return T;
+  };
+  static_assert(!KT || (TA && !TB && !SEG), "K-block table: transposed-A weight gradients only");
+  auto kt_set = [&](const Tile& T, int slab) {
+    if constexpr (KT) {
+      const long row = kt_row(T.k_begin / BK + slab);
+      kt_dA = row * p.lda; kt_dB = row * p.ldb;
+    }
   };
   const long stepA = TA ? (long)BK * p.lda : (long)BK, stepB = TB ? (long)BK : (long)BK * p.ldb;
   auto issue = [&](const Tile& T, int slab, int stage) {
@@ -308,6 +326,9 @@
     if constexpr (SEG) {
       issue_from<128>(sA, T.sa, seg_tab[0][slab], w);
       issue_from<BN_>(sB, T.sb, seg_tab[1][slab], w);
+    } else if constexpr (KT) {
+      issue_from<128>(sA, T.sa, kt_dA, w);
+      issue_from<BN_>(sB, T.sb, kt_dB, w);
     } else {
       issue_from<128>(sA, T.sa, slab * stepA, w);
       issue_from<BN_>(sB, T.sb, slab * stepB, w);
@@ -319,14 +340,15 @@
     char* sB = sA + A_BYTES;
     long dA_, dB_;
     if constexpr (SEG) { dA_ = seg_tab[0][slab]; dB_ = seg_tab[1][slab]; }
+    else if constexpr (KT) { dA_ = kt_dA; dB_ = kt_dB; }
     else { dA_ = slab * stepA; dB_ = slab * stepB; }
     if (q < 4) glds16(T.sa[q] + dA_, sA + __builtin_amdgcn_readfirstlane((w * 4 + q) * 1024));
     else glds16(T.sb[q - 4] + dB_, sB + __builtin_amdgcn_readfirstlane((w * (BN_ / 32) + (q - 4)) * 1024));
   };
   Tile cur = tile_of(0);
   if (cur.nfull < 0) return;
-  if (cur.nfull > 0) issue(cur, 0, 0);
-  if (cur.nfull > 1) issue(cur, 1, 1);
+  if (cur.nfull > 0) { kt_set(cur, 0); issue(cur, 0, 0); }
+  if (cur.nfull > 1) { kt_set(cur, 1); issue(cur, 1, 1); }
   bool drained = false;
 
   for (int it = 0;; ++it) {
@@ -378,6 +400,7 @@
     if constexpr (NST == 3) {
       for (int s = 0; s < n; ++s) {
         const int stage = s % 3;
+        if (s + 2 < n) kt_set(cur, s + 2);
         if (!(drained && s < 2)) {
           if (s + 1 < n) { if (GI == 8) asm volatile("s_waitcnt vmcnt(8)" ::: "memory"); else asm volatile("s_waitcnt vmcnt(6)" ::: "memory"); }
           else asm volatile("s_waitcnt vmcnt(0)" ::: "memory");
@@ -394,6 +417,7 @@
   #ifdef TFASR_GEMM_TIMING
         long long tp = __builtin_readcyclecounter();
   #endif
+        if (s + 2 < n) kt_set(cur, s + 2);
         if (!(drained && s < 2)) {
           if (s + 1 < n) { if (GI == 8) asm volatile("s_waitcnt vmcnt(8)" ::: "memory"); else asm volatile("s_waitcnt vmcnt(6)" ::: "memory"); }
           else asm volatile("s_waitcnt vmcnt(0)" ::: "memory");
@@ -427,9 +451,10 @@
     if (cur.tail) {
       char* sA = smem;
       char* sB = smem + A_BYTES;
-      const int kt = cur.k_begin + n * BK;
-      if (TA) tail_trans<128>(sA, cur.A, p.lda, cur.m0, p.M, kt, cur.k_end); else tail_direct<128>(sA, cur.A, p.lda, cur.m0, p.M, kt, cur.k_end);
-      if (TB) tail_direct<BN_>(sB, cur.B, p.ldb, cur.n0, p.N, kt, cur.k_end); else tail_trans<BN_>(sB, cur.B, p.ldb, cur.n0, p.N, kt, cur.k_end);
+      const int kt = KT ? (int)kt_row(cur.k_begin / BK + n) : cur.k_begin + n * BK;
+      const int ke = KT ? p.K : cur.k_end;
+      if (TA) tail_trans<128>(sA, cur.A, p.lda, cur.m0, p.M, kt, ke); else tail_direct<128>(sA, cur.A, p.lda, cur.m0, p.M, kt, ke);
+      if (TB) tail_direct<BN_>(sB, cur.B, p.ldb, cur.n0, p.N, kt, ke); else tail_trans<BN_>(sB, cur.B, p.ldb, cur.n0, p.N, kt, ke);
       __syncthreads();
       mma_slab<TA, TB, BN_, C_CS>(sA, sB, wm, wn, lane, acc, accb, do_cs);
       __syncthreads();
@@ -439,8 +464,8 @@
     if constexpr (ONE) nxt.nfull = -1;
     else {
       nxt = tile_of(it + 1);
-      if (nxt.nfull > 0) issue(nxt, 0, 0);
-      if (nxt.nfull > 1) issue(nxt, 1, 1);
+      if (nxt.nfull > 0) { kt_set(nxt, 0); issue(nxt, 0, 0); }
+      if (nxt.nfull > 1) { kt_set(nxt, 1); issue(nxt, 1, 1); }
     }
 #ifdef TFASR_GEMM_TIMING
     const long long t_main = __builtin_readcyclecounter();
@@ -743,6 +768,11 @@
   gemm_fast_body<TA, TB, 128, 0, 2, false, true>(p, gx, gy, gz, ntiles, (int)blockIdx.x, (int)gridDim.x);
 }
 
+template <int EPI>
+__global__ __launch_bounds__(256, 2) void gemm_ktab_kernel(const tfasr_gemm_args p, const int gx, const int gy, const int gz, const int ntiles) {
+  gemm_fast_body<true, false, 128, EPI, 2, false, false, false, true>(p, gx, gy, gz, ntiles, (int)blockIdx.x, (int)gridDim.x);
+}
+
 constexpr int GROUP_MAX = 10;
 constexpr int GROUP_UNITS = 20;
 struct GroupArgs {
@@ -752,7 +782,7 @@
   int j0[8][GROUP_UNITS + 1];
   int nunit[8];
 };
-template <int EPI, int NST, int BN_>
+template <int EPI, int NST, int BN_, bool KT = false>
 __global__ __launch_bounds__(256, 2) void wgrad_group_kernel(const GroupArgs ga) {
   const int x = blockIdx.x & 7, j = blockIdx.x >> 3;
   const int nu = ga.nunit[x];
@@ -763,7 +793,7 @@
   if (u < 0) return;
   const int q = ga.uq[x][u], ks = ga.uks[x][u], t = j - ga.j0[x][u];
   const tfasr_gemm_args* pp = ga.p + q;
-  gemm_fast_body<true, false, BN_, EPI, NST, true>(*pp, ga.gx[q], ga.gy[q], 1, ga.gx[q] * ga.gy[q], t, ks);
+  gemm_fast_body<true, false, BN_, EPI, NST, true, false, false, KT>(*pp, ga.gx[q], ga.gy[q], 1, ga.gx[q] * ga.gy[q], t, ks);
 }
 
 __global__ __launch_bounds__(256) void splitk_reduce_kernel(const float* __restrict__ ws, float* __restrict__ D, int M, int N, int ldd, int split) {
@@ -793,6 +823,10 @@
 }
 
 int num_cus();
+inline bool ktab_eligible(const tfasr_gemm_args& a) {
+  return a.dtype == TFASR_BF16 && a.trans_a && !a.trans_b && a.accumulate && a.nb1 * a.nb2 <= 1 && !a.ws && !a.seg_a_off && !a.row_tiles && !a.lse_part &&
+         !a.rgrad_coef && !a.bns_out && a.n_k_tiles > 0 && a.n_k_tiles <= (a.K + 255) / 256;
+}
 
 int num_cus() {
   static int n = 0;
@@ -834,6 +868,23 @@
 template <bool TA, bool TB>
 int launch_one(const tfasr_gemm_args& a, hipStream_t stream) {
   const int split = a.split_k > 1 ? a.split_k : 1;
+  if (a.k_tiles) {
+    if constexpr (TA && !TB) {
+      if (ktab_eligible(a) && a.out_f32) {
+        dim3 grid((a.N + 127) / 128, (a.M + BM - 1) / BM, split);
+        if ((long)grid.x * grid.y * grid.z > 0x7fffffffL) return TFASR_STATUS_INVALID_VALUE;
+        const long ntiles = (long)grid.x * grid.y * grid.z;
+        const int slots = 2 * num_cus();
+        int G = (int)(ntiles < slots ? ntiles : slots);
+        if (ntiles >= slots) G &= ~7;
+        constexpr int SMEM = 2 * (A_BYTES + 128 * BK * 2) + 4 * (64 / (128 / 16)) * (128 / 2 + 4) * 4;
+        TFASR_KLAUNCH((gemm_ktab_kernel<E_CSUM>), dim3(G), dim3(256), SMEM, stream, a, (int)grid.x, (int)grid.y, (int)grid.z, (int)ntiles);
+        TFASR_CHECK_LAUNCH();
+        return TFASR_STATUS_SUCCESS;
+      }
+    }
+    return TFASR_STATUS_UNSUPPORTED;
+  }
   static const bool bn64_off = false;
   const long t128 = (long)((a.N + 127) / 128) * ((a.M + BM - 1) / BM) * a.nb1 * a.nb2 * split;
   static const long bn64_thr = (1L << 40);
@@ -947,7 +998,7 @@
 bool group_eligible(const tfasr_gemm_args& a) {
   return a.dtype == TFASR_BF16 && a.trans_a && !a.trans_b && a.accumulate && a.out_f32 && a.nb1 * a.nb2 <= 1 && !a.ws && !a.bias && !a.res &&
          !a.dact_z && !a.prez && a.act == TFASR_ACT_NONE && a.drop_p == 0.f && al16(a.A) && al16(a.B) && !(a.lda & 7) && !(a.ldb & 7) &&
-         ((a.M + 7) & ~7) <= a.lda && ((a.N + 7) & ~7) <= a.ldb && a.K >= 8 && a.N > 64 && a.M > 0;
+         ((a.M + 7) & ~7) <= a.lda && ((a.N + 7) & ~7) <= a.ldb && a.K >= 8 && a.N > 64 && a.M > 0 && (!a.k_tiles || ktab_eligible(a));
 }
 
 }
@@ -957,7 +1008,9 @@
 int tfasr_gemm_group_fast_try(const tfasr_gemm_args* a, int n, hipStream_t stream) {
   if (n < 2 || n > GROUP_MAX) return TFASR_STATUS_UNSUPPORTED;
   for (int i = 0; i < n; ++i)
-    if (!group_eligible(a[i])) return TFASR_STATUS_UNSUPPORTED;
+    if (!group_eligible(a[i]) || (a[i].k_tiles != nullptr) != (a[0].k_tiles != nullptr)) return TFASR_STATUS_UNSUPPORTED;
+  const bool ktab = a[0].k_tiles != nullptr;
+  auto keff = [](const tfasr_gemm_args& g) -> long { return g.k_tiles ? 256L * g.n_k_tiles : (long)g.K; };
   GroupArgs ga;
   memset(&ga, 0, sizeof(ga));
   long total = 0;
@@ -969,7 +1022,7 @@
   }
   static const long env_slots = 0;
   long kmax = 0;
-  for (int i = 0; i < n; ++i) kmax = a[i].K > kmax ? a[i].K : kmax;
+  for (int i = 0; i < n; ++i) kmax = keff(a[i]) > kmax ? keff(a[i]) : kmax;
   const long slots = env_slots > 0 ? env_slots : ((g_tfasr_group_beside || kmax >= 131072) ? num_cus() * 5L / 4 : 2L * num_cus());
   long split = slots / (total > 0 ? total : 1);
   if (split < 1) split = 1;
@@ -983,7 +1036,7 @@
   int nu = 0;
   for (int i = 0; i < n; ++i) {
     long sp = split;
-    if (a[i].K / 512 < sp) sp = a[i].K / 512;
+    if (keff(a[i]) / 512 < sp) sp = keff(a[i]) / 512;
     if (sp < 1) sp = 1;
     if (sp > 64) sp = 64;
     ga.p[i] = a[i];
@@ -1021,7 +1074,8 @@
     else TFASR_KLAUNCH((wgrad_group_kernel<E_CSUM, 2, 64>), dim3(8 * maxload), dim3(256), 2 * STAGE, stream, ga);
   } else {
     constexpr int STAGE = A_BYTES + 128 * BK * 2;
-    TFASR_KLAUNCH((wgrad_group_kernel<E_CSUM, 2, 128>), dim3(8 * maxload), dim3(256), 2 * STAGE, stream, ga);
+    if (ktab) TFASR_KLAUNCH((wgrad_group_kernel<E_CSUM, 2, 128, true>), dim3(8 * maxload), dim3(256), 2 * STAGE, stream, ga);
+    else TFASR_KLAUNCH((wgrad_group_kernel<E_CSUM, 2, 128>), dim3(8 * maxload), dim3(256), 2 * STAGE, stream, ga);
   }
   TFASR_CHECK_LAUNCH();
   return TFASR_STATUS_SUCCESS;
diff --git a/tensorflowasr_amd/kernels.py b/tensorflowasr_amd/kernels.py
--- a/tensorflowasr_amd/kernels.py
+++ b/tensorflowasr_amd/kernels.py
@@ -244,9 +244,10 @@
 
 def gemm(A, B, out, M, N, K, lda, ldb, ldd, trans_a=False, trans_b=False, bias=None, res=None, dact_z=None,
          prez=None, alpha=1.0, beta=1.0, act=ACT_NONE, dact=ACT_NONE, nb1=1, nb2=1, sA=(0, 0), sB=(0, 0), sD=(0, 0),
-         accumulate=False, split_k=1, drop_p=0.0, drop_seed=0, colsum=None, lse=None, seg=None, rgrad=None, bns=None, row_tiles=None):
+         accumulate=False, split_k=1, drop_p=0.0, drop_seed=0, colsum=None, lse=None, seg=None, rgrad=None, bns=None, row_tiles=None,
+         k_tiles=None):
     a = _gemm_args(A, B, out, M, N, K, lda, ldb, ldd, trans_a, trans_b, bias, res, dact_z, prez, alpha, beta, act, dact, nb1, nb2, sA, sB, sD,
-                   accumulate, split_k, drop_p, drop_seed, colsum)
+                   accumulate, split_k, drop_p, drop_seed, colsum, k_tiles)
     if rgrad is not None:
         coef, row_label = rgrad
         assert coef.dtype == torch.float32 and coef.is_contiguous() and row_label.dtype == torch.int32
@@ -268,8 +269,8 @@
         assert part.dtype == torch.float32 and pick.dtype == torch.float32 and row_label.dtype == torch.int32
         a.lse_part, a.lse_parts, a.row_label, a.pick = part.data_ptr(), part.shape[1], row_label.data_ptr(), pick.data_ptr()
     st = _lib.load().tfasr_gemm(ctypes.byref(a), _stream())
-    if (lse is not None or seg is not None or rgrad is not None or bns is not None) and st == _lib.STATUS_UNSUPPORTED:
-        raise _lib.TfasrUnsupported("gemm: fused row statistics / K-segments / gradient epilogue are not available for this product")
+    if (lse is not None or seg is not None or rgrad is not None or bns is not None or k_tiles is not None) and st == _lib.STATUS_UNSUPPORTED:
+        raise _lib.TfasrUnsupported("gemm: fused row statistics / K-segments / gradient epilogue / K-block table are not available for this product")
     check(st, "gemm")
     return out
 
@@ -278,12 +279,15 @@
     arr = (GemmArgs * len(calls))()
     for i, kw in enumerate(calls):
         arr[i] = _gemm_args(**kw)
-    check(_lib.load().tfasr_gemm_group(arr, len(calls), _stream()), "gemm_group")
+    st = _lib.load().tfasr_gemm_group(arr, len(calls), _stream())
+    if st == _lib.STATUS_UNSUPPORTED and any(kw.get("k_tiles") is not None for kw in calls):
+        raise _lib.TfasrUnsupported("gemm_group: K-block table not available for these products")
+    check(st, "gemm_group")
 
 
 def _gemm_args(A, B, out, M, N, K, lda, ldb, ldd, trans_a=False, trans_b=False, bias=None, res=None, dact_z=None,
                prez=None, alpha=1.0, beta=1.0, act=ACT_NONE, dact=ACT_NONE, nb1=1, nb2=1, sA=(0, 0), sB=(0, 0), sD=(0, 0),
-               accumulate=False, split_k=1, drop_p=0.0, drop_seed=0, colsum=None):
+               accumulate=False, split_k=1, drop_p=0.0, drop_seed=0, colsum=None, k_tiles=None):
     a = GemmArgs()
     a.A, a.B, a.D = A.data_ptr(), B.data_ptr(), (out.data_ptr() if out is not None else None)
     a.bias = bias.data_ptr() if bias is not None else None
@@ -304,9 +308,12 @@
     a.split_k = split_k
     a.drop_p, a.drop_seed = drop_p, drop_seed
     a.colsum = colsum.data_ptr() if colsum is not None else None
+    if k_tiles is not None:
+        assert k_tiles.dtype == torch.int32 and k_tiles.is_cuda and k_tiles.is_contiguous()
+        a.k_tiles, a.n_k_tiles = k_tiles.data_ptr(), k_tiles.numel()
     if accumulate:
         assert out.dtype == torch.float32
-        if _SPLITK_WS and split_k > 1 and nb1 * nb2 == 1:
+        if _SPLITK_WS and split_k > 1 and nb1 * nb2 == 1 and k_tiles is None:
             ws = workspace(4 * split_k * M * N, out.device, "splitk_%d" % (_raw_stream(torch.cuda.current_device()) if _raw_stream else 0))
             a.ws, a.ws_elems = ws.data_ptr(), ws.numel() // 4
     return a
@@ -910,10 +917,11 @@
     check(_L().tfasr_conv1_stats_from_gram(_p(gram), _p(w), _p(bias), _p(stats), w.shape[-1], _stream()), "conv1_stats_from_gram")
 
 
-def conv1_bn_bwd_onepass_s2d(x, w, bias, fin, dy, bstats, pbuf):
+def conv1_bn_bwd_onepass_s2d(x, w, bias, fin, dy, bstats, pbuf, row_list=None):
     B, T0, F0 = x.shape[:3]
-    check(_L().tfasr_conv1_bn_bwd_onepass_s2d(_p(x), _p(w), _p(bias), _p(fin), _p(dy), _p(bstats), _p(pbuf), B, T0, F0, w.shape[-1], _dt(x),
-                                              _stream()), "conv1_bn_bwd_onepass")
+    assert row_list is None or (row_list.dtype == torch.int32 and row_list.is_cuda and row_list.is_contiguous())
+    check(_L().tfasr_conv1_bn_bwd_onepass_s2d_rows(_p(x), _p(w), _p(bias), _p(fin), _p(dy), _p(bstats), _p(pbuf), B, T0, F0, w.shape[-1], _dt(x),
+                                                   _p(row_list), 0 if row_list is None else row_list.numel(), _stream()), "conv1_bn_bwd_onepass")
 
 
 def conv1_bn_bwd_finalize(gram, w, bias, fin, bstats, count, pbuf, dw, db):
@@ -936,6 +944,16 @@
     if st == _lib.STATUS_UNSUPPORTED:
         raise _lib.TfasrUnsupported("s2d_tail_fill: bf16 tensors with C % 8 == 0 only")
     check(st, "s2d_tail_fill")
+    return x
+
+
+def s2d_tail_fold(x, r_tt, scratch, B, T2, F2, C):
+    assert r_tt.dtype == torch.int32 and r_tt.is_cuda and r_tt.numel() == B
+    assert scratch.dtype == torch.float32 and scratch.is_cuda and scratch.numel() >= B * (F2 + 1) * C
+    st = _L().tfasr_s2d_tail_fold(_p(x), _p(r_tt), _p(scratch), B, T2, F2, C, _dt(x), _stream())
+    if st == _lib.STATUS_UNSUPPORTED:
+        raise _lib.TfasrUnsupported("s2d_tail_fold: bf16 tensors with C % 8 == 0 only")
+    check(st, "s2d_tail_fold")
     return x
 
 
```

Result: faster. 5.023 audio-hours/sec, median of 6 (+3.7%).
